# BGU-CS-VIL/DPMMSubClusters.jl

Hardware: AMD Instinct MI355X
Metric: Gibbs iterations/sec, N=10M D=64 NIW (higher is better)
Workload: dtype f32

## Files before the change

### dpmmsubclusters.jl_amd/binding.py

```python
import ctypes
import os
import subprocess

import numpy as np

_HERE = os.path.dirname(os.path.abspath(__file__))
PRIOR_NIW, PRIOR_MULT = 0, 1
MAX_CLUSTERS = 1024

_c_i64p = ctypes.POINTER(ctypes.c_int64)
_c_f32p = ctypes.POINTER(ctypes.c_float)
_c_f64p = ctypes.POINTER(ctypes.c_double)

ABI = [
    ("dpmm_abi_version", ctypes.c_int, []),
    ("dpmm_create", ctypes.c_int, [ctypes.POINTER(ctypes.c_void_p), ctypes.c_int, ctypes.c_int, ctypes.c_int64, ctypes.c_int64, ctypes.c_int, ctypes.c_uint64]),
    ("dpmm_destroy", ctypes.c_int, [ctypes.c_void_p]),
    ("dpmm_last_error", ctypes.c_char_p, [ctypes.c_void_p]),
    ("dpmm_upload_points", ctypes.c_int, [ctypes.c_void_p, _c_f32p, ctypes.c_int64]),
    ("dpmm_upload_points_device", ctypes.c_int, [ctypes.c_void_p, ctypes.c_void_p, ctypes.c_int64]),
    ("dpmm_upload_points_npy", ctypes.c_int, [ctypes.c_void_p, ctypes.c_void_p, ctypes.c_int, ctypes.c_int64, ctypes.c_int]),
    ("dpmm_upload_points_csc", ctypes.c_int, [ctypes.c_void_p, _c_i64p, _c_i64p, _c_f32p, ctypes.c_int]),
    ("dpmm_init_labels", ctypes.c_int, [ctypes.c_void_p, ctypes.c_int, ctypes.c_uint32]),
    ("dpmm_set_labels", ctypes.c_int, [ctypes.c_void_p, _c_i64p, _c_i64p]),
# ... 20 lines not shown
    ("dpmm_mult_master_draw", ctypes.c_int, [ctypes.c_void_p, ctypes.c_uint32, ctypes.c_int, ctypes.c_int, ctypes.c_void_p, ctypes.c_void_p]),
    ("dpmm_mult_master_draws", ctypes.c_int, [ctypes.c_void_p, ctypes.c_int, ctypes.c_void_p]),
    ("dpmm_mult_master_put_rows", ctypes.c_int, [ctypes.c_void_p, ctypes.c_void_p, ctypes.c_int]),
    ("dpmm_mult_master_pairs_ahead", ctypes.c_int, [ctypes.c_void_p, ctypes.c_int, ctypes.c_void_p, ctypes.c_void_p, ctypes.c_int]),
    ("dpmm_mult_master_marginals", ctypes.c_int, [ctypes.c_void_p, ctypes.c_int, ctypes.POINTER(ctypes.c_void_p), ctypes.POINTER(ctypes.c_void_p), ctypes.POINTER(ctypes.c_int)]),
    ("dpmm_mult_master_rows_on_demand", ctypes.c_int, [ctypes.c_void_p, ctypes.c_int]),
    ("dpmm_mult_master_rows_wait", ctypes.c_int, [ctypes.c_void_p]),
    ("dpmm_sweep", ctypes.c_int, [ctypes.c_void_p, ctypes.c_uint32, ctypes.c_int]),
    ("dpmm_packed_stride", ctypes.c_int64, [ctypes.c_void_p]),
    ("dpmm_suffstats_packed_device", ctypes.c_int, [ctypes.c_void_p, _c_i64p, ctypes.c_int, ctypes.c_void_p]),
    ("dpmm_suffstats_packed", ctypes.c_int, [ctypes.c_void_p, _c_i64p, ctypes.c_int, _c_f64p]),
    ("dpmm_unpack_suffstats", ctypes.c_int, [ctypes.c_void_p, ctypes.c_int, _c_f64p, _c_f64p, _c_f64p, _c_f64p]),
    ("dpmm_split", ctypes.c_int, [ctypes.c_void_p, _c_i64p, _c_i64p, ctypes.c_int, ctypes.c_uint32]),
    ("dpmm_merge", ctypes.c_int, [ctypes.c_void_p, _c_i64p, _c_i64p, ctypes.c_int]),
    ("dpmm_remove_empty", ctypes.c_int, [ctypes.c_void_p, _c_i64p, ctypes.c_int]),
    ("dpmm_reset_sublabels", ctypes.c_int, [ctypes.c_void_p, _c_i64p, ctypes.c_int, ctypes.c_uint32]),
    ("dpmm_set_predictive_niw", ctypes.c_int, [ctypes.c_void_p, ctypes.c_int, _c_f32p, _c_f32p, _c_f32p, _c_f32p, _c_f32p]),
    ("dpmm_set_predictive_mult", ctypes.c_int, [ctypes.c_void_p, ctypes.c_int, _c_f32p, _c_f32p]),
    ("dpmm_predict", ctypes.c_int, [ctypes.c_void_p, _c_f32p]),
    ("dpmm_predict_points", ctypes.c_int, [ctypes.c_void_p, _c_i64p, _c_f32p]),
    ("dpmm_set_ground_truth", ctypes.c_int, [ctypes.c_void_p, _c_i64p, ctypes.c_int]),
    ("dpmm_contingency", ctypes.c_int, [ctypes.c_void_p, ctypes.c_int, _c_i64p]),
    ("dpmm_bin_counts", ctypes.c_int, [ctypes.c_void_p, _c_i64p]),
    ("dpmm_smart_project", ctypes.c_int, [ctypes.c_void_p, ctypes.c_int64, _c_f64p, _c_f64p, _c_f64p, _c_i64p]),
    ("dpmm_smart_kmeans_iter", ctypes.c_int, [ctypes.c_void_p, ctypes.c_int64, ctypes.c_double, ctypes.c_double, _c_f64p]),
    ("dpmm_smart_assign", ctypes.c_int, [ctypes.c_void_p, ctypes.c_int64, ctypes.c_double, ctypes.c_double]),
    ("dpmm_debug_loglik", ctypes.c_int, [ctypes.c_void_p, _c_f32p]),
    ("dpmm_sync", ctypes.c_int, [ctypes.c_void_p]),
    ("dpmm_stream", ctypes.c_void_p, [ctypes.c_void_p]),
    ("dpmm_last_sweep_parts_ms", ctypes.c_int, [ctypes.c_void_p, _c_f32p]),
    ("dpmm_last_kernel_ms", ctypes.c_int, [ctypes.c_void_p, _c_f32p, _c_f32p]),
    ("dpmm_debug_counters", ctypes.c_int, [ctypes.c_void_p, ctypes.POINTER(ctypes.c_int64), ctypes.c_int]),
    ("dpmm_debug_sort_tables", ctypes.c_int, [ctypes.c_void_p, ctypes.c_void_p, ctypes.c_void_p, ctypes.c_void_p, ctypes.c_void_p]),
    ("dpmm_debug_set_prelaunch_hook", ctypes.c_int, [ctypes.c_void_p, ctypes.c_void_p]),
    ("dpmm_init_labels_from", ctypes.c_int, [ctypes.c_void_p, ctypes.c_int, ctypes.c_int, ctypes.c_uint32]),
    ("dpmm_set_option", ctypes.c_int, [ctypes.c_void_p, ctypes.c_int, ctypes.c_double]),
    ("dpmm_params_staging", ctypes.c_int, [ctypes.c_void_p, ctypes.c_int] + [ctypes.POINTER(ctypes.c_void_p)] * 6),
    ("dpmm_commit_params", ctypes.c_int, [ctypes.c_void_p, ctypes.c_int]),
    ("dpmm_suffstats_host", ctypes.c_int, [ctypes.c_void_p, _c_i64p, ctypes.c_int, ctypes.POINTER(ctypes.c_void_p)]),
    ("dpmm_step_stats", ctypes.c_int, [ctypes.c_void_p, ctypes.c_uint32, ctypes.POINTER(ctypes.c_void_p), ctypes.POINTER(ctypes.c_void_p)]),
    ("dpmm_debug_subloglik", ctypes.c_int, [ctypes.c_void_p, _c_f32p]),
    ("dpmm_debug_ref_bracket", ctypes.c_int, [ctypes.c_void_p, ctypes.c_int64, ctypes.c_float, _c_f32p, _c_f32p]),
    ("dpmm_debug_pair_ball", ctypes.c_int, [ctypes.c_void_p, _c_f32p, _c_f32p]),
    ("dpmm_debug_pair_ball_sn2", ctypes.c_int, [ctypes.c_void_p, _c_f32p]),
    ("dpmm_debug_norm_cert_points", ctypes.c_int, [ctypes.c_void_p, ctypes.c_int, ctypes.POINTER(ctypes.c_uint8)]),
    ("dpmm_debug_bracket_big", ctypes.c_int, [ctypes.c_void_p, _c_f32p, ctypes.POINTER(ctypes.c_uint32)]),
    ("dpmm_debug_mult_draws_ahead", ctypes.c_int, [ctypes.c_void_p, ctypes.POINTER(ctypes.c_longlong)]),
    ("dpmm_last_sweep_work", ctypes.c_int, [ctypes.c_void_p, ctypes.POINTER(ctypes.c_uint64)]),
    ("dpmm_comm_use_library", ctypes.c_int, [ctypes.c_char_p]),
    ("dpmm_comm_unique_id", ctypes.c_int, [ctypes.c_void_p]),
    ("dpmm_comm_init", ctypes.c_int, [ctypes.c_void_p, ctypes.c_void_p, ctypes.c_int, ctypes.c_int]),
    ("dpmm_comm_init_host", ctypes.c_int, [ctypes.c_void_p, ctypes.c_int, ctypes.c_int, ctypes.c_void_p, ctypes.c_void_p]),
    ("dpmm_comm_info", ctypes.c_int, [ctypes.c_void_p, _c_i64p]),
    ("dpmm_last_comm_ms", ctypes.c_int, [ctypes.c_void_p, _c_f32p, _c_f32p]),
    ("dpmm_comm_destroy", ctypes.c_int, [ctypes.c_void_p]),
    ("dpmm_comm_allgather_host", ctypes.c_int, [ctypes.c_void_p, ctypes.c_void_p, ctypes.c_int64, ctypes.c_void_p]),
]

ABI_TENSOR = [
    ("dpmm_upload_points_strided_device", ctypes.c_int, [ctypes.c_void_p, ctypes.c_void_p, ctypes.c_int, ctypes.c_int64, ctypes.c_int64, ctypes.c_int]),
    ("dpmm_get_points_device", ctypes.c_int, [ctypes.c_void_p, ctypes.c_void_p, ctypes.c_int64]),
    ("dpmm_get_labels_device", ctypes.c_int, [ctypes.c_void_p, ctypes.c_void_p, ctypes.c_void_p]),
    ("dpmm_set_labels_device", ctypes.c_int, [ctypes.c_void_p, ctypes.c_void_p, ctypes.c_void_p]),
    ("dpmm_predict_points_device", ctypes.c_int, [ctypes.c_void_p, ctypes.c_void_p, ctypes.c_void_p]),
]
_c_f64p_in = ctypes.POINTER(ctypes.c_double)
# ... 1215 lines not shown
        self._chk(self._lib.dpmm_debug_loglik(self._h, _p(out, _c_f32p)))
        return out

    def sync(self):
        self._chk(self._lib.dpmm_sync(self._h))

    @property
    def stream(self):
        return self._lib.dpmm_stream(self._h)

    def set_timing(self, on):
        mask = 7 if on is True else int(on)
        self.timing = mask != 0
        self.set_option(OPT_KERNEL_TIMING, float(mask))

    def last_sweep_parts_ms(self):
        out = np.zeros(3, np.float32)
        self._chk(self._lib.dpmm_last_sweep_parts_ms(self._h, _p(out, _c_f32p)))
        return [float(v) for v in out]

    def last_kernel_ms(self):
        if not self.timing:
            raise RuntimeError("kernel timing is off for this Worker (timing=False / set_timing(False)): no events were recorded")
        a = ctypes.c_float(); b = ctypes.c_float()
        self._chk(self._lib.dpmm_last_kernel_ms(self._h, ctypes.byref(a), ctypes.byref(b)))
        return a.value, b.value

    def debug_sort_tables(self):
        perm = np.empty(max(self.n, 1), np.int32); tot = np.empty(2 * self.K, np.int32); start = np.empty(2 * self.K + 1, np.int32)
        ptot = np.zeros(1, np.int32)
        self._chk(self._lib.dpmm_debug_sort_tables(self._h, perm.ctypes.data, tot.ctypes.data, start.ctypes.data, ptot.ctypes.data))
        return perm[:int(ptot[0])].copy(), tot, start

    def debug_counters(self):
        out = (ctypes.c_int64 * 4)()
        self._chk(self._lib.dpmm_debug_counters(self._h, out, 4))
        return list(out)
```

### dpmmsubclusters.jl_amd/csrc/dpmm_api.cpp

```cpp
#include "../../include/dpmm_hip.h"
#include "../../include/dpmm_hip_master.h"
#include "../../include/dpmm_hip_debug.h"
#include "../../include/dpmm_hip_tensor.h"
#include "../../include/dpmm_hip_csc.h"
#include "../../include/dpmm_hip_score.h"
#include "../../include/dpmm_hip_rank.h"
#include "../../include/dpmm_hip_overlap.h"
#include "../../include/dpmm_hip_batchstats.h"
#include "../../include/dpmm_hip_countstats.h"
#include "../../include/dpmm_hip_typicality.h"
#include "../../include/dpmm_hip_explain.h"
#include "../../include/dpmm_hip_holdout.h"
#include "../../include/dpmm_hip_countholdout.h"
#include "../../include/dpmm_hip_trace.h"
#include "../../include/dpmm_hip_missing.h"
#include "../../include/dpmm_hip_impute.h"
#include "../../include/dpmm_hip_regress.h"
#include "../../include/dpmm_hip_regress_draw.h"
#include "../../include/dpmm_hip_regress_cdf.h"
#include "../../include/dpmm_hip_recommend.h"
#include "../../include/dpmm_hip_sample.h"
#include "../../include/dpmm_hip_project.h"

#include <hip/hip_runtime.h>
// ... 15 lines not shown
#include <vector>

#include "dpmm_kernels.h"
#include "project_image.h"
#include "typicality_math.h"
#include "dev_mem.h"

namespace dpmm {
void (*g_prelaunch)(void *) = nullptr;
void *g_prelaunch_arg = nullptr;
}
using namespace dpmm;

static_assert(DPMM_MAX_CLUSTERS == DPMM_MAX_CLUSTERS_K, "header / kernel limits out of sync");

#ifdef DPMM_STAMPS
static unsigned long long *g_dbg = nullptr;
#endif
namespace {
thread_local std::string g_create_error;

int nb_for_dim(int D) { return D <= 16 ? 1 : D <= 32 ? 2 : D <= 64 ? 4 : D <= 128 ? 8 : 16; }
}

struct AccSession {
    bool active = false;
    int K = 0, mode = 0, floor = 0;
    float min_logdens = 0.f;
    unsigned long long gen = 0;
    int use2 = 0;
    float min2 = 0.f;
    bool accumulated = false;
};

struct dpmm_ctx {
    int prior = 0, D = 0, device = 0;
    int64_t n = 0, first = 0, ldx = 0;
    uint64_t seed = 0;
    int NB = 0;
    int tile = 0;
    int64_t ntiles = 0;
    int cus = 256;
    int sweep_grid = 0, sweep_grid_max = 0;
    hipStream_t stream = nullptr;
    hipEvent_t ev[4] = {nullptr, nullptr, nullptr, nullptr};
    hipEvent_t ev_part[2] = {nullptr, nullptr};
    int have_parts = 0;
    bool have_sweep_ev = false, have_stats_ev = false;

    DevBuf<float> dX;
    DevBuf<int32_t> dbins;
    bool have_points = false, have_labels = false;
    DevBuf<int32_t> d_gt;
    int n_gt = 0;
    DevBuf<unsigned long long> d_cont;
    bool have_perm = false;

    int K = 0, Kcap = 0;
    DevBuf<float> d_raw;
    DevBuf<float> d_mu;
    DevBuf<float> d_Rp;
    DevBuf<float> d_mup;
    DevBuf<float> d_cst;
    DevBuf<uint32_t> d_Lp16;
    DevBuf<float> d_raw2, d_Rp2;
    DevBuf<uint32_t> d_Lp16_2;
// ... 183 lines not shown
    uint32_t noise_epoch = 0;
    int noise_nmat = 0, noise_buf = 0;
    bool spec_inflight = false, spec_valid = false;
    uint32_t spec_epoch = 0;
    std::vector<int32_t> spec_slots;
    DevBuf<int32_t> d_jobs, d_dslots;
    PinBuf<int32_t> h_list[4];
    int h_list_next = 0;
    std::vector<int32_t> jobs_shadow, dslots_shadow;
    PinBuf<uint8_t> h_master;
    bool draws_on_device = false;
    DevBuf<unsigned long long> d_work;
    int work_waves = 0;
    long long work_launches = 0;
    float opt_margin = 50.f;
    int opt_prio = 1;
    int opt_queue_rounds = -1;
    int opt_ball = 1;
    DevBuf<uint32_t> d_sp_frag;
    DevBuf<uint32_t> d_refb_big;
    bool have_refb_big = false;
    DevBuf<uint32_t> d_brk_flag;
    DevBuf<float> d_brk_aref;
    DevBuf<float> d_sp_cons;
    PinBuf<uint32_t> h_need;
    int opt_direction = -1;
    bool sp_ready = false, sp_regime = false;
    unsigned sp_count = 0;
    bool sp_last = false;
    int sp_K = -1;
    int sp_cooldown = 0;
    int opt_b3 = 1;
    bool have_b3 = false;
    int opt_chain = 0x7fffffff & ~(8 | 32);
    DevBuf<uint8_t> d_cert_rec;
    int opt_lean_norm_cert = 1;
    int opt_pair_ball = 1;
    bool have_pb = false;
    int opt_lean_dir = 1;
    int opt_master_poll = 1;
    int opt_lean = 1;
    DevBuf<uint32_t> d_hard;
    int hard_flip = 0;
    int perm_nbins = 0;
    PinBuf<uint32_t> h_hard;
    bool sn2_tight = false;
    bool cert_fb = false;
    int cert_cool = 0;
    int lean_off = 0;
    bool lean_ran = false;
    int lean_backoff = 15;
    int opt_bf16scr = 1;
    int opt_bracket = 1;
    int opt_timing = 0;
    int opt_tail = 1, opt_prescreen = -1, opt_ordered = 1, opt_force_f32 = 0, opt_trace = 0, opt_ref_const = 0;
    int64_t opt_stats_items = 0;
    int opt_stats_groups = 0;
    void *comm = nullptr;
    int rank = 0, world = 1;
    dpmm_host_allreduce_fn host_fn = nullptr;
    void *host_user = nullptr;
    PinBuf<char> h_red;
    hipEvent_t ev_comm[4] = {nullptr, nullptr, nullptr, nullptr};
    bool have_comm_ev[2] = {false, false};
    int64_t comm_bytes[2] = {0, 0};
    int64_t comm_calls = 0;
    int comm_timeout_ms = 1800000;
// ... 40 lines not shown
}
static inline void wd_arm(dpmm_ctx *c) {
    std::lock_guard<std::mutex> lk(c->wd_mu);
    c->wd_wait_since.store(steady_ms() | 1, std::memory_order_relaxed);
}
static inline bool wd_disarm(dpmm_ctx *c) {
    std::lock_guard<std::mutex> lk(c->wd_mu);
    c->wd_wait_since.store(0, std::memory_order_relaxed);
    if (c->comm_aborted.load() && !c->abort_reported) { c->abort_reported = true; return true; }
    return false;
}
static inline hipError_t sync_stream(dpmm_ctx *c, hipStream_t st) {
    if (st == c->stream) c->sync_gen += 1;
    if (!c->watchdog || !c->coll_pending) return hipStreamSynchronize(st);
    wd_arm(c);
    hipError_t e = hipStreamSynchronize(st);
    if (wd_disarm(c)) e = hipErrorLaunchTimeOut;
    else if (e == hipSuccess && st == c->stream) c->coll_pending = false;
    return e;
}
static inline hipError_t sync_event(dpmm_ctx *c, hipEvent_t ev) {
    if (!c->watchdog || !c->coll_pending) return hipEventSynchronize(ev);
    wd_arm(c);
    hipError_t e = hipEventSynchronize(ev);
    if (wd_disarm(c)) e = hipErrorLaunchTimeOut;
    return e;
}

static int fail(dpmm_ctx *c, int code, const std::string &msg) {
    if (c) c->err = msg; else g_create_error = msg;
    return code;
}

template <class Buf>
static int regrow(dpmm_ctx *c, Buf &buf, size_t need, const char *who, const char *what, size_t floor = 0) {
    const size_t cap = grow_capacity(need, floor);
    if (buf.alloc(cap) != hipSuccess)
        return fail(c, DPMM_EHIP, std::string(who) + ": out of device memory for the " + what + " (" + std::to_string((unsigned long long)cap) + " bytes)");
    return DPMM_OK;
}
template <class Buf>
static inline int grow(dpmm_ctx *c, Buf &buf, size_t need, const char *who, const char *what, size_t floor = 0) {
    if (need <= buf.bytes) return DPMM_OK;
    HIPCHK(c, sync_stream(c, c->stream));
    return regrow(c, buf, need, who, what, floor);
}
template <typename T>
static int sampler_table(dpmm_ctx *c, DevBuf<T> &dst, const T *src, size_t bytes) {
    HIPCHK(c, dst.alloc(bytes));
    HIPCHK(c, hipMemcpy(dst, src, bytes, hipMemcpyHostToDevice));
    return DPMM_OK;
}
static inline int ensure_pinned(dpmm_ctx *c, size_t bytes) { return grow(c, c->h_pin, bytes, "dpmm", "pinned staging block", (size_t)1 << 20); }

struct UidByValue { char internal[128]; };
namespace {
struct Rccl {
    void *handle = nullptr;
    int (*GetUniqueId)(void *) = nullptr;
    int (*CommInitRank)(void **, int,  UidByValue, int) = nullptr;
    int (*CommDestroy)(void *) = nullptr;
    int (*CommAbort)(void *) = nullptr;
    int (*AllReduce)(const void *, void *, size_t, int, int, void *, hipStream_t) = nullptr;
    int (*AllGather)(const void *, void *, size_t, int, void *, hipStream_t) = nullptr;
    const char *(*GetErrorString)(int) = nullptr;
    std::string err;
// ... 183 lines not shown
    if (prior_kind == DPMM_PRIOR_NIW) {
        c->NB = nb_for_dim(D);
        c->tile = niw_tile_points(c->NB);
        c->slab_stride = niw_slab_stride(D);
        c->packed_stride = 1 + (int64_t)D + (int64_t)D * (D + 1) / 2;
        c->sweep_grid = c->cus * niw_occupancy(c->NB);
        CHK_CREATE(c->d_row_off.alloc(sizeof(int32_t) * (size_t)c->packed_stride));
        CHK_CREATE(c->d_inv_off.alloc(sizeof(int32_t) * (size_t)c->slab_stride));
        CHK_CREATE(launch_niw_row_offsets(c->d_row_off, c->d_inv_off, D, c->packed_stride, c->stream));
    } else {
        c->tile = mult_tile_points();
        c->slab_stride = mult_slab_stride(D);
        c->packed_stride = 1 + (int64_t)D;
        c->sweep_grid = c->cus * 2;
    }
    c->ntiles = (n_local + c->tile - 1) / c->tile;
    if (c->ntiles < c->sweep_grid) c->sweep_grid = (int)std::max<int64_t>(1, c->ntiles);
    c->sweep_grid_max = c->sweep_grid;
    const int64_t target_items = (c->prior == DPMM_PRIOR_NIW && c->D <= 64) ? 16384 : 8192;
    const int64_t min_chunk = (c->prior == DPMM_PRIOR_NIW && c->D <= 64) ? 32 : 256;
    const int64_t target_items2 = (c->prior == DPMM_PRIOR_NIW && c->D <= 64) ? 65536 : target_items;
    c->chunk = (int)std::max<int64_t>(min_chunk, ((n_local + target_items2 - 1) / target_items2 + 3) / 4 * 4);
    c->chunk_dense = c->chunk;
    const size_t nalloc = (size_t)std::max<int64_t>(n_local, 1);
    if (prior_kind == DPMM_PRIOR_NIW) CHK_CREATE(c->dX.alloc(sizeof(float) * nalloc * (size_t)c->ldx));
    CHK_CREATE(c->dbins.alloc(sizeof(int32_t) * nalloc));
    c->sb.tile = n_local <= 4000000 ? SORT_TILE_SMALL : SORT_TILE;
    const int alloc_tile = c->sb.tile;
    c->sort_tile_min = alloc_tile;
    c->nt_sort = (int)((n_local + alloc_tile - 1) / alloc_tile);
    const size_t nbmax = 2 * DPMM_MAX_CLUSTERS;
    CHK_CREATE(c->sort_mem.tile_hist.alloc(sizeof(int32_t) * nbmax * (size_t)std::max(1, c->nt_sort)));
    CHK_CREATE(c->sort_mem.tile_cnt.alloc(sizeof(int32_t) * nbmax * (size_t)std::max(1, c->nt_sort)));
    CHK_CREATE(c->sort_mem.tile_spec.alloc(sizeof(int32_t) * (size_t)STEP_SPEC_MAX_BINS * (size_t)std::max(1, c->nt_sort)));
    CHK_CREATE(c->sort_mem.spec_bins.alloc(sizeof(int32_t) * nalloc));
    CHK_CREATE(c->sort_mem.fast_total.alloc(sizeof(int32_t) * nbmax * FAST_TOTAL_STRIDE));
    CHK_CREATE(hipMemsetAsync(c->sort_mem.fast_total, 0, sizeof(int32_t) * nbmax * FAST_TOTAL_STRIDE, c->stream));
    CHK_CREATE(c->sort_mem.ticket.alloc(sizeof(unsigned)));
    CHK_CREATE(hipMemsetAsync(c->sort_mem.ticket, 0, sizeof(unsigned), c->stream));
    CHK_CREATE(c->sort_mem.prev_lab.alloc(sizeof(uint16_t) * (((size_t)nalloc + SORT_TILE - 1) / SORT_TILE * SORT_TILE)));
    CHK_CREATE(hipMemsetAsync(c->sort_mem.prev_lab, 0xFF, sizeof(uint16_t) * (((size_t)nalloc + SORT_TILE - 1) / SORT_TILE * SORT_TILE), c->stream));
    CHK_CREATE(c->sort_mem.cdirty.alloc(DPMM_MAX_CLUSTERS + 8));
    CHK_CREATE(hipMemsetAsync(c->sort_mem.cdirty, 1, DPMM_MAX_CLUSTERS + 8, c->stream));
    CHK_CREATE(c->sort_mem.cmode.alloc(DPMM_MAX_CLUSTERS));
    CHK_CREATE(hipMemsetAsync(c->sort_mem.cmode, 0, DPMM_MAX_CLUSTERS, c->stream));
    CHK_CREATE(c->sort_mem.bin_total.alloc(sizeof(int32_t) * nbmax));
    CHK_CREATE(c->sort_mem.bin_start.alloc(sizeof(int32_t) * (nbmax + 1)));
    CHK_CREATE(c->sort_mem.item_start.alloc(sizeof(int32_t) * (nbmax + 1)));
    CHK_CREATE(c->sort_mem.perm.alloc(sizeof(int32_t) * nalloc));
    CHK_CREATE(c->sort_mem.bin_sel.alloc(nbmax));
    c->sel_capacity = (int)nbmax;
    CHK_CREATE(c->sort_mem.perm_total.alloc(sizeof(int32_t)));
    sort_view(c);
    CHK_CREATE(c->d_small.alloc(sizeof(int32_t) * 4 * DPMM_MAX_CLUSTERS));
    CHK_CREATE(c->d_counts64.alloc(sizeof(long long) * 2 * DPMM_MAX_CLUSTERS));
    CHK_CREATE(c->d_cside.alloc(DPMM_MAX_CLUSTERS));
    CHK_CREATE(hipMemsetAsync(c->d_cside, 0, DPMM_MAX_CLUSTERS, c->stream));
    if (c->prior == DPMM_PRIOR_NIW && c->NB == 4) {
        CHK_CREATE(c->d_sp_frag.alloc(sizeof(uint32_t) * (size_t)SP_MAXK * SP_FRAG_WORDS));
        CHK_CREATE(c->d_sp_cons.alloc(sizeof(float) * (size_t)SP_MAXK * SP_CONS_FLOATS));
        CHK_CREATE(c->h_need.alloc(sizeof(uint32_t) * 20 * (size_t)std::max(1, c->sweep_grid_max)));
        memset(c->h_need, 0, sizeof(uint32_t) * 20 * (size_t)std::max(1, c->sweep_grid_max));
        if (c->NB == 4) {
            const size_t hw = hard_list_words(n_local);
            CHK_CREATE(c->d_hard.alloc(sizeof(uint32_t) * 2 * hw));
            CHK_CREATE(hipMemsetAsync(c->d_hard, 0, sizeof(uint32_t) * 2 * hw, c->stream));
// ... 201 lines not shown
            if (e == hipSuccess) e = hipMemcpyAsync(n_cp, ncp.data(), sizeof(int64_t) * ((size_t)n + 1), hipMemcpyHostToDevice, c->stream);
            if (e == hipSuccess) e = launch_csc_compact(t_cp, t_rv, t_nz, n, index_base, n_cp, n_ri, n_val, c->stream);
            if (e == hipSuccess) e = sync_stream(c, c->stream);
        }
    } else if (e == hipSuccess) {
        e = hipMemsetAsync(n_cp, 0, sizeof(int64_t), c->stream);
        if (e == hipSuccess) e = sync_stream(c, c->stream);
    }
    if (e != hipSuccess || rc != DPMM_OK) {
        if (e != hipSuccess) return fail(c, DPMM_EHIP, std::string("dpmm_upload_points_csc: ") + hipGetErrorString(e));
        return fail(c, rc, msg);
    }
    t_cp.reset(); t_rv.reset(); t_nz.reset(); t_cnt.reset(); t_bad.reset();
    c->dX.reset(); c->dX8.reset();
    c->d_cp = std::move(n_cp); c->d_ri = std::move(n_ri); c->d_val = std::move(n_val); c->nnz = ncp[n];
    c->x_sparse = 1; c->x_u8 = 0; c->x_bf16_exact = 0; c->repack_pending = false;
    if (int rc2 = set_points_chunk(c, true)) return rc2;
    if (c->have_params && c->d_raw) {
        if (int rc2 = pack_sparse_image(c, c->d_raw, c->d_Rp, c->K)) return rc2;
        c->rp_current = false;
        c->mspec_valid = false;
        HIPCHK(c, sync_stream(c, c->stream));
    }
    c->have_points = true;
    c->cache_force = true;
    c->rows_full_K = -1;
    return DPMM_OK;
}

int dpmm_init_labels(dpmm_ctx *c, int init_clusters, uint32_t epoch) {
    if (!c) return DPMM_EINVAL;
    if (init_clusters < 1 || init_clusters > DPMM_MAX_CLUSTERS) return fail(c, DPMM_ELIMIT, "init_clusters out of range");
    HIPCHK(c, hipSetDevice(c->device));
    if (c->n > 0) HIPCHK(c, launch_init_labels(c->dbins, c->n, c->first, init_clusters, 0, c->seed, epoch, c->stream));
    c->have_labels = true;
    c->rows_full_K = -1;
    return DPMM_OK;
}

int dpmm_init_labels_from(dpmm_ctx *c, int init_clusters, int first_label, uint32_t epoch) {
    if (!c) return DPMM_EINVAL;
    if (first_label < 1 || init_clusters < 1 || first_label - 1 + init_clusters > DPMM_MAX_CLUSTERS) return fail(c, DPMM_ELIMIT, "init_clusters / first_label out of range");
    HIPCHK(c, hipSetDevice(c->device));
    if (c->n > 0) HIPCHK(c, launch_init_labels(c->dbins, c->n, c->first, init_clusters, first_label - 1, c->seed, epoch, c->stream));
    c->have_labels = true;
    c->rows_full_K = -1;
    return DPMM_OK;
}

int dpmm_set_labels(dpmm_ctx *c, const int64_t *labels, const int64_t *sub) {
    if (!c) return DPMM_EINVAL;
    if (!c->have_labels && (!labels || !sub)) return fail(c, DPMM_ESTATE, "first dpmm_set_labels must provide both vectors");
    HIPCHK(c, hipSetDevice(c->device));
    if (c->n == 0) { c->have_labels = true; return DPMM_OK; }
    DevBuf<int64_t> tmp;
    HIPCHK(c, tmp.alloc(sizeof(int64_t) * 2 * (size_t)c->n));
    int rc = DPMM_OK;
    hipError_t e = hipSuccess;
    if (labels) e = hipMemcpyAsync(tmp, labels, sizeof(int64_t) * c->n, hipMemcpyHostToDevice, c->stream);
    if (e == hipSuccess && sub) e = hipMemcpyAsync(tmp + c->n, sub, sizeof(int64_t) * c->n, hipMemcpyHostToDevice, c->stream);
    if (e == hipSuccess) e = launch_bins_from_i64(c->dbins, labels ? tmp.get() : nullptr, sub ? tmp + c->n : nullptr, c->n, c->stream);
    if (e == hipSuccess) e = sync_stream(c, c->stream);
    if (e != hipSuccess) { c->err = std::string("dpmm_set_labels: ") + hipGetErrorString(e); rc = DPMM_EHIP; }
    else c->have_labels = true;
    c->rows_full_K = -1;
    return rc;
}

int dpmm_get_labels(dpmm_ctx *c, int64_t *labels, int64_t *sub) {
    if (!c) return DPMM_EINVAL;
    if (!c->have_labels) return fail(c, DPMM_ESTATE, "labels not initialised");
    HIPCHK(c, hipSetDevice(c->device));
    if (c->n == 0) return DPMM_OK;
    DevBuf<int64_t> tmp;
    HIPCHK(c, tmp.alloc(sizeof(int64_t) * 2 * (size_t)c->n));
    hipError_t e = launch_bins_to_i64(c->dbins, tmp, tmp + c->n, c->n, c->stream);
    if (e == hipSuccess && labels) e = hipMemcpyAsync(labels, tmp, sizeof(int64_t) * c->n, hipMemcpyDeviceToHost, c->stream);
    if (e == hipSuccess && sub) e = hipMemcpyAsync(sub, tmp + c->n, sizeof(int64_t) * c->n, hipMemcpyDeviceToHost, c->stream);
    if (e == hipSuccess) e = sync_stream(c, c->stream);
    if (e != hipSuccess) { c->err = std::string("dpmm_get_labels: ") + hipGetErrorString(e); return DPMM_EHIP; }
    return DPMM_OK;
}

static int check_K(dpmm_ctx *c, int K) {
    if (K < 1) return fail(c, DPMM_EINVAL, "K < 1");
    if (K > DPMM_MAX_CLUSTERS) return fail(c, DPMM_ELIMIT, "K > DPMM_MAX_CLUSTERS");
    return DPMM_OK;
}

struct ParLayout {
    size_t mu = 0, mat = 0, logdet = 0, lr = 0, w = 0, cst = 0, slot = 0, bytes = 0;
};
static ParLayout par_layout(const dpmm_ctx *c, int slots) {
// ... 306 lines not shown
        }
        HIPCHK(c, launch_niw_bracket_big(c->NB, a, c->d_refb_big, c->d_brk_flag, c->d_brk_aref, c->stream));
        a.brk_flag = c->d_brk_flag; a.brk_aref = c->d_brk_aref;
    }
    a.work = table ? nullptr : c->d_work;
    if (!table) { c->work_waves = std::max(c->work_waves, 4 * c->sweep_grid); c->work_launches += 1; }
    a.prio = c->opt_prio; a.queue_rounds = c->opt_queue_rounds;
#ifdef DPMM_STAMPS
    if (!g_dbg) { hipMalloc(&g_dbg, sizeof(unsigned long long) * 16 * 4 * 4096); hipMemset(g_dbg, 0, sizeof(unsigned long long) * 16 * 4 * 4096); }
    a.dbg = g_dbg;
#endif
    return DPMM_OK;
}

static bool lean_this_sweep(dpmm_ctx *c, const NiwSweepArgs &a) {
    const bool lean_ok = c->opt_lean != 0 && c->opt_bracket && a.use_prev && a.screen_margin > 0.f && !a.final_argmax && a.lam == nullptr && c->K > 1 && c->d_hard &&
                         !(c->opt_lean_dir == 0 && c->sp_regime && c->opt_direction != 0 && c->sp_ready);
    if (!lean_ok) return false;
    if (c->lean_off == 0 && c->lean_ran) {
        const int64_t nwt = (c->n + 63) / 64;
        if ((int64_t)c->h_hard[0] * 10 > nwt * 3) { c->lean_off = c->lean_backoff; c->lean_backoff = std::min(2 * c->lean_backoff + 1, 1023); }
        else c->lean_backoff = 15;
        c->lean_ran = false;
    }
    if (c->lean_off > 0) { c->lean_off -= 1; c->h_hard[0] = 0; return false; }
    c->lean_ran = true;
    return true;
}

static int niw_label_store_chain(dpmm_ctx *c, const NiwSweepArgs &a, bool use_lean) {
    const bool parts = (c->opt_timing & 8) != 0 && (c->opt_timing & 1) != 0;
    if (parts && !c->ev_part[0]) for (auto &e : c->ev_part) HIPCHK(c, hipEventCreate(&e));
    NiwLabelStore ls{true};
    if (use_lean) {
        const size_t hw = hard_list_words(c->n);
        uint32_t *mine = c->d_hard + (size_t)c->hard_flip * hw, *other = c->d_hard + (size_t)(c->hard_flip ^ 1) * hw;
        c->hard_flip ^= 1;
        uint32_t *need2 = a.need ? need_lean_settled(c) : nullptr, *need3 = a.need ? need_lean_dir(c) : nullptr;
        const bool al = a.order != nullptr && c->perm_nbins > 0 && c->perm_nbins <= NIW_LEAN_MAX_BINS;
        NiwSweepArgs al_args = a;
        if (!c->opt_lean_dir) { al_args.sp_frag = nullptr; al_args.sp_cons = nullptr; }
        if (c->have_pb && c->opt_pair_ball && al_args.ball) {
            al_args.ball |= NIW_BALL_PAIR_TABLE;
            if (c->opt_lean_norm_cert) al_args.ball |= NIW_BALL_NORM_CERT;
            if (c->opt_lean_norm_cert == 3) al_args.ball |= NIW_BALL_NB_LOOSE;
        }
        c->cert_fb = need2 != nullptr && (al_args.ball & NIW_BALL_NORM_CERT) != 0 && !(al_args.sp_frag && al_args.sp_cons);
#ifndef DPMM_STAMPS
        al_args.cert_points = c->d_cert_rec;
#endif
        HIPCHK(c, launch_niw_lean(al_args, mine, need2, other, al ? c->sb.bin_start : nullptr, al ? c->perm_nbins : 0, need3, c->sweep_grid, c->stream));
        if (parts) HIPCHK(c, hipEventRecord(c->ev_part[0], c->stream));
        ls.tile_list = mine;
        ls.list_len = c->h_hard;
    }
    HIPCHK(c, launch_niw_sweep(c->NB, a, c->sweep_grid, c->stream, ls));
    if (parts) HIPCHK(c, hipEventRecord(c->ev_part[1], c->stream));
    c->have_parts = parts ? (use_lean ? 2 : 1) : 0;
    if (!ls.tile_list) HIPCHK(c, launch_niw_sub(a, nullptr, nullptr, c->sweep_grid, c->stream));
    return DPMM_OK;
}

static int run_sweep(dpmm_ctx *c, uint32_t epoch, int final_argmax, float *table, int64_t table_stride, int64_t p0 = 0, int64_t np = -1) {
    if (!c->have_points || !c->have_params) return fail(c, DPMM_ESTATE, "sweep needs points and parameters");
    HIPCHK(c, hipSetDevice(c->device));
    if (c->n == 0) return DPMM_OK;
    const bool ranged = np >= 0;
    if (ranged && (!table || p0 < 0 || p0 % c->tile != 0 || np == 0 || p0 + np > c->n)) return fail(c, DPMM_EINVAL, "run_sweep: bad point range");
    const int64_t rn = ranged ? np : c->n;
    const int64_t rtiles = ranged ? (np + c->tile - 1) / c->tile : c->ntiles;
    const int rgrid = ranged ? (int)std::min<int64_t>(c->sweep_grid, rtiles) : c->sweep_grid;
    if (c->prior == DPMM_PRIOR_NIW && !table) {
        if (!c->work_zeroed) HIPCHK(c, hipMemsetAsync(c->d_work, 0, sizeof(unsigned long long) * DPMM_WORK_SLOTS, c->stream));
        c->work_zeroed = false;
    }
    if (!table && (c->opt_timing & 1)) HIPCHK(c, hipEventRecord(c->ev[0], c->stream));
    if (c->prior == DPMM_PRIOR_NIW) {
        NiwSweepArgs a{};
        if (int rc = niw_sweep_args(c, a, epoch, final_argmax, table, table_stride, ranged, p0, rn, rtiles)) return rc;
        const bool b3 = c->NB == 4 && c->have_b3 && c->opt_b3 && !table && !c->predictive && a.tail != nullptr;
        if (b3) {
            if (int rc = niw_label_store_chain(c, a, lean_this_sweep(c, a))) return rc;
        } else {
            HIPCHK(c, launch_niw_sweep(c->NB, a, rgrid, c->stream));
            if (!table) c->have_parts = 0;
        }
    } else {
        MultSweepArgs a{};
        a.X = (ranged && c->dX) ? c->dX + p0 * c->ldx : c->dX; a.ldx = c->ldx; a.n = rn; a.first_index = c->first + p0; a.D = c->D; a.K = c->K;
        a.logp = c->d_Rp; a.cst = c->d_cst;
        a.scratch = table ? table : c->d_scratch;
        a.scratch_stride = table ? table_stride : c->scratch_stride;
// ... 120 lines not shown
    if (c->n == 0) return DPMM_OK;
    const int64_t stride = c->ntiles * c->tile;
    const int rows = (c->prior == DPMM_PRIOR_NIW) ? c->K : 3 * c->K;
    DevBuf<float> table;
    HIPCHK(c, table.alloc(sizeof(float) * (size_t)rows * (size_t)stride));
    int rc = run_sweep(c, 0, 0, table, stride);
    if (rc == DPMM_OK) {
        const size_t src_pitch = sizeof(float) * stride * (c->prior == DPMM_PRIOR_MULT ? 3 : 1);
        hipError_t e = hipMemcpy2DAsync(out, sizeof(float) * c->n, table, src_pitch, sizeof(float) * c->n,
                                        (size_t)c->K, hipMemcpyDeviceToHost, c->stream);
        if (e == hipSuccess) e = sync_stream(c, c->stream);
        if (e != hipSuccess) { c->err = std::string("dpmm_debug_loglik: ") + hipGetErrorString(e); rc = DPMM_EHIP; }
        else if (c->opt_ref_const && c->prior == DPMM_PRIOR_NIW && !c->predictive) {
            const float k2pi = (float)(-0.5 * (double)c->D * (double)c->D * log(2.0 * M_PI));
            for (size_t i = 0; i < (size_t)c->K * (size_t)c->n; ++i) out[i] += k2pi;
        }
    }
    return rc;
}

int64_t dpmm_packed_stride(const dpmm_ctx *c) { return c ? c->packed_stride : 0; }

static inline int ensure_out(dpmm_ctx *c, size_t bytes) {
    if (bytes <= c->h_out.bytes) return DPMM_OK;
    HIPCHK(c, sync_stream(c, c->stream));
    c->rows_late = false;
    return regrow(c, c->h_out, bytes, "dpmm", "pinned statistics rows", (size_t)1 << 20);
}

static int flush_undo(dpmm_ctx *c) {
    if (!c->undo_pending) return DPMM_OK;
    c->undo_pending = false;
    const uint8_t *flags = reinterpret_cast<const uint8_t *>(c->d_out.get()) + sizeof(double) * 2 * (size_t)c->K * (size_t)c->packed_stride;
    HIPCHK(c, launch_niw_undo_reset(c->dbins, c->n, c->K, flags, c->d_cside, c->stream));
    return DPMM_OK;
}
static int run_stats(dpmm_ctx *c, const int64_t *idx, int n_idx, bool with_reset = false, uint32_t reset_epoch = 0, uint8_t *flags_to = nullptr,
                     bool *flags_sent = nullptr) {
    if (!c->have_points || !c->have_labels || c->K < 1) return fail(c, DPMM_ESTATE, "suffstats need points, labels and parameters (K)");
    HIPCHK(c, hipSetDevice(c->device));
    const int nbins = 2 * c->K;
    c->marg_valid = false;
    c->mspec_valid = false;
    const bool one_auto = c->packed_stride <= 4096;
    const bool one_coll = with_reset && comm_attached(c) && (c->opt_one_collective < 0 ? one_auto : c->opt_one_collective != 0);
    c->last_pass_one_collective = one_coll;
    if (c->opt_timing & 2) HIPCHK(c, hipEventRecord(c->ev[2], c->stream));
    if (idx) {
        c->h_sel.assign(nbins, 0);
        for (int j = 0; j < n_idx; ++j) {
            if (idx[j] < 1 || idx[j] > c->K) return fail(c, DPMM_EINVAL, "cluster index out of range");
            c->h_sel[2 * (idx[j] - 1)] = 1;
            c->h_sel[2 * (idx[j] - 1) + 1] = 1;
        }
        if (int rc = ensure_pinned(c, nbins + 8)) return rc;
        HIPCHK(c, sync_stream(c, c->stream));
        memcpy(c->h_pin, c->h_sel.data(), nbins);
        HIPCHK(c, launch_copy_bytes(c->sb.bin_sel, c->h_pin, nbins, c->stream));
        c->sel_all_ones = 0;
    } else if (with_reset && c->n > 0 && c->opt_derive) {
    } else if (c->sel_all_ones < nbins) {
        HIPCHK(c, hipMemsetAsync(c->sb.bin_sel, 1, c->sel_capacity, c->stream));
        c->sel_all_ones = c->sel_capacity;
    }
    bool derive = false;
    StatsArgs a{};
    a.X = c->dX; a.ldx = c->ldx; a.n = c->n; a.D = c->D; a.nbins = nbins; a.chunk = c->chunk;
    a.max_items = (int)((c->n + c->chunk - 1) / c->chunk) + nbins;
    a.range_groups = c->opt_stats_groups;
    a.sb = c->sb; a.slabs = c->d_slabs; a.slab_stride = c->slab_stride; a.out = (one_coll && c->prior == DPMM_PRIOR_NIW) ? c->d_red : c->d_out; a.packed_stride = c->packed_stride; a.row_off = c->d_row_off; a.inv_off = c->d_inv_off;
    if (with_reset && c->n > 0) {
        const bool fold_reset = (c->opt_chain & 8) != 0 && (c->n >= 4000000 || (c->opt_chain & 32) != 0) && nbins <= STEP_SPEC_MAX_BINS &&
                                c->sb.tile_spec != nullptr && c->sb.spec_bins != nullptr;
        HIPCHK(c, launch_step_hist(c->dbins, c->n, nbins, c->sb, c->stream, fold_reset ? 1 : 0, c->first, c->seed, reset_epoch));
        const long long *gc = nullptr;
        if (comm_attached(c) && !one_coll) {
            HIPCHK(c, launch_widen_counts(c->sb.fast_total, FAST_TOTAL_STRIDE, c->d_counts64, nbins, c->stream));
            if (int rc = comm_allreduce(c, c->d_counts64, nbins, 0)) return rc;
            gc = c->d_counts64;
        }
        uint8_t *flags = reinterpret_cast<uint8_t *>(c->d_out.get()) + sizeof(double) * (size_t)nbins * (size_t)c->packed_stride;
        if (!fold_reset) HIPCHK(c, launch_step_reset(c->dbins, c->n, c->first, nbins, c->sb, gc, flags, c->K, c->seed, reset_epoch, one_coll ? c->d_cside : nullptr, c->stream));
        derive = c->opt_derive != 0;
        const int force_all = (c->cache_force || c->cache_K != c->K) ? 1 : 0;
        const StepReset rs{gc, flags, c->K, one_coll ? c->d_cside : nullptr, c->first, c->seed, reset_epoch};
        HIPCHK(c, launch_step_scan_scatter(c->dbins, a, derive ? 1 : 0, force_all, c->opt_chain & 1, fold_reset ? &rs : nullptr, c->stream));
        if (derive) { c->sel_all_ones = 0; c->cache_force = false; c->cache_K = c->K; }
    } else {
        if (c->n > 0) {
            HIPCHK(c, launch_sort_by_bin(c->dbins, c->n, nbins, c->sb, c->stream));
        } else {
            HIPCHK(c, hipMemsetAsync(c->sb.bin_total, 0, sizeof(int32_t) * nbins, c->stream));
        }
        if (with_reset && one_coll) {
            HIPCHK(c, hipMemsetAsync(c->d_cside, 0, (size_t)c->K, c->stream));
        } else if (with_reset) {
            const long long *gc = nullptr;
            if (comm_attached(c)) {
                HIPCHK(c, launch_widen_counts(c->sb.bin_total, 1, c->d_counts64, nbins, c->stream));
                if (int rc = comm_allreduce(c, c->d_counts64, nbins, 0)) return rc;
                gc = c->d_counts64;
            }
            uint8_t *flags = reinterpret_cast<uint8_t *>(c->d_out.get()) + sizeof(double) * (size_t)nbins * (size_t)c->packed_stride;
            HIPCHK(c, launch_bad_flags(c->sb.bin_total, gc, c->K, flags, c->stream));
        }
        HIPCHK(c, launch_sort_finish(c->dbins, a, c->stream));
    }
    c->have_perm = c->n > 0;
    c->perm_nbins = nbins;
    if (flags_sent) *flags_sent = false;
    if (one_coll) {
        uint8_t *flags = reinterpret_cast<uint8_t *>(c->d_out.get()) + sizeof(double) * (size_t)nbins * (size_t)c->packed_stride;
        const size_t nred = 3 * (size_t)c->K * (size_t)c->packed_stride;
        if (c->n > 0 && c->prior == DPMM_PRIOR_NIW) {
            if (derive) { a.mode = c->sb.cmode; a.cache = c->d_ccache; a.dirty = c->sb.cdirty; a.K = c->K; }
            a.cside = c->d_cside; a.zero2 = flags + c->K;
            HIPCHK(c, launch_niw_stats(a, c->stream));
        } else if (c->n > 0) {
            if (c->x_sparse) HIPCHK(c, launch_mult_stats_sparse(a, sparse_args(c), c->stream));
            else if (c->x_u8) HIPCHK(c, launch_mult_stats_u8(a, c->dX8, c->ld8, c->stream));
            else HIPCHK(c, launch_mult_stats(a, c->stream));
            if (derive) HIPCHK(c, launch_derive_rows(c->d_out, c->d_ccache, c->sb.cmode, c->sb.cdirty, c->packed_stride, c->K, flags, nullptr, c->stream));
// ... 14 lines not shown
        return DPMM_OK;
    }
    const bool ride = derive && flags_to != nullptr && !comm_attached(c);
    const uint8_t *fsrc = reinterpret_cast<const uint8_t *>(c->d_out.get()) + sizeof(double) * (size_t)nbins * (size_t)c->packed_stride;
    if (c->prior == DPMM_PRIOR_NIW) {
        if (derive) {
            a.mode = c->sb.cmode; a.cache = c->d_ccache; a.dirty = c->sb.cdirty; a.K = c->K;
            a.flags_src = ride ? fsrc : nullptr; a.flags_dst = ride ? flags_to : nullptr;
        }
        HIPCHK(c, launch_niw_stats(a, c->stream));
    } else {
        if (c->x_sparse) HIPCHK(c, launch_mult_stats_sparse(a, sparse_args(c), c->stream));
        else if (c->x_u8) HIPCHK(c, launch_mult_stats_u8(a, c->dX8, c->ld8, c->stream));
        else HIPCHK(c, launch_mult_stats(a, c->stream));
        if (derive) HIPCHK(c, launch_derive_rows(c->d_out, c->d_ccache, c->sb.cmode, c->sb.cdirty, c->packed_stride, c->K, fsrc, ride ? flags_to : nullptr, c->stream));
    }
    if (ride && flags_sent) *flags_sent = true;
    if (comm_attached(c)) {
        if (int rc = comm_allreduce(c, c->d_out, (size_t)nbins * (size_t)c->packed_stride, 1)) return rc;
    }
    if (c->opt_timing & 2) HIPCHK(c, hipEventRecord(c->ev[3], c->stream));
    c->have_stats_ev = (c->opt_timing & 2) != 0;
    c->rows_full_K = idx ? -1 : c->K;
    return DPMM_OK;
}

int dpmm_bin_counts(dpmm_ctx *c, int64_t *counts) {
    if (!c || !counts) return DPMM_EINVAL;
    if (!c->have_points || !c->have_labels || c->K < 1) return fail(c, DPMM_ESTATE, "bin counts need points, labels and parameters (K)");
    HIPCHK(c, hipSetDevice(c->device));
    const int nbins = 2 * c->K;
    if (c->n == 0) { for (int b = 0; b < nbins; ++b) counts[b] = 0; return DPMM_OK; }
    if (int rc = ensure_pinned(c, sizeof(int32_t) * nbins)) return rc;
    HIPCHK(c, launch_sort_by_bin(c->dbins, c->n, nbins, c->sb, c->stream));
    HIPCHK(c, launch_copy_bytes(c->h_pin, c->sb.bin_total, sizeof(int32_t) * nbins, c->stream));
    HIPCHK(c, sync_stream(c, c->stream));
    const int32_t *h = reinterpret_cast<const int32_t *>(c->h_pin.get());
    for (int b = 0; b < nbins; ++b) counts[b] = h[b];
    return DPMM_OK;
}

int dpmm_suffstats_packed_device(dpmm_ctx *c, const int64_t *idx, int n_idx, double *d_out) {
    if (!c || !d_out) return DPMM_EINVAL;
    if (int rc = run_stats(c, idx, n_idx)) return rc;
    HIPCHK(c, hipMemcpyAsync(d_out, c->d_out, sizeof(double) * 2 * c->K * (size_t)c->packed_stride, hipMemcpyDeviceToDevice, c->stream));
    HIPCHK(c, sync_stream(c, c->stream));
    return DPMM_OK;
}

int dpmm_suffstats_host(dpmm_ctx *c, const int64_t *idx, int n_idx, const double **packed) {
    if (!c || !packed) return DPMM_EINVAL;
    const size_t out_bytes = sizeof(double) * 2 * (size_t)std::max(c->K, 1) * (size_t)c->packed_stride;
    if (int rc = ensure_out(c, out_bytes + DPMM_MAX_CLUSTERS + 64)) return rc;
    if (int rc = run_stats(c, idx, n_idx)) return rc;
    HIPCHK(c, launch_copy_bytes(c->h_out, c->d_out, out_bytes, c->stream));
    HIPCHK(c, sync_stream(c, c->stream));
    *packed = reinterpret_cast<const double *>(c->h_out.get());
    return DPMM_OK;
}

static int mult_marginals_launch(dpmm_ctx *c);
int dpmm_step_stats(dpmm_ctx *c, uint32_t reset_epoch, const double **packed, const uint8_t **bad) {
    if (!c || !packed || !bad) return DPMM_EINVAL;
    const size_t out_bytes = sizeof(double) * 2 * (size_t)std::max(c->K, 1) * (size_t)c->packed_stride;
    if (int rc = ensure_out(c, out_bytes + DPMM_MAX_CLUSTERS + 64)) return rc;
    const bool maybe_late = c->rows_on_demand && c->marg_req && c->opt_mult_draws_ahead && c->mdraw_seen && c->draws_on_device && c->d_raw2;
// ... 205 lines not shown
            else if (now - drained > std::chrono::seconds(5)) { rc = fail(c, DPMM_EHIP, "posterior records missing 5 s after the stream drained"); break; }
        } else if (q != hipErrorNotReady) { c->err = std::string("hipStreamQuery while waiting for the posteriors: ") + hipGetErrorString(q); rc = DPMM_EHIP; break; }
    }
    if (armed && wd_disarm(c)) {
        c->err = "collective timed out: a peer rank is gone or stuck (communicator aborted after DPMM_OPT_COMM_TIMEOUT_MS)";
        return DPMM_ECOMM;
    }
    if (c->comm_aborted.load(std::memory_order_relaxed) && rc == DPMM_OK && master_records_marked(sm, nrec)) return fail(c, DPMM_ECOMM, "communicator aborted");
    return rc;
}

int dpmm_debug_set_prelaunch_hook(void (*fn)(void *), void *arg) {
    dpmm::g_prelaunch_arg = arg;
    dpmm::g_prelaunch = fn;
    return DPMM_OK;
}

int dpmm_debug_counters(dpmm_ctx *c, int64_t *out, int n) {
    if (!c || !out || n < 1) return DPMM_EINVAL;
    for (int i = 0; i < n; ++i) out[i] = 0;
    out[0] = c->dbg_early_wait;
    return DPMM_OK;
}

int dpmm_debug_sort_tables(dpmm_ctx *c, int32_t *perm, int32_t *bin_total, int32_t *bin_start, int32_t *perm_total) {
    if (!c || !perm || !bin_total || !bin_start || !perm_total) return DPMM_EINVAL;
    if (!c->have_perm || c->K < 1) return fail(c, DPMM_ESTATE, "no statistics pass has sorted the points yet");
    HIPCHK(c, hipSetDevice(c->device));
    HIPCHK(c, hipStreamSynchronize(c->stream));
    HIPCHK(c, hipMemcpy(perm, c->sb.perm, sizeof(int32_t) * (size_t)c->n, hipMemcpyDeviceToHost));
    HIPCHK(c, hipMemcpy(bin_total, c->sb.bin_total, sizeof(int32_t) * 2 * (size_t)c->K, hipMemcpyDeviceToHost));
    HIPCHK(c, hipMemcpy(bin_start, c->sb.bin_start, sizeof(int32_t) * (2 * (size_t)c->K + 1), hipMemcpyDeviceToHost));
    HIPCHK(c, hipMemcpy(perm_total, c->sb.perm_total, sizeof(int32_t), hipMemcpyDeviceToHost));
    return DPMM_OK;
}

int dpmm_step_master_device(dpmm_ctx *c, uint32_t reset_epoch, const int32_t *slots, uint32_t draw_epoch, const uint8_t **bad, const double **small) {
    if (!c || !slots || !bad || !small) return DPMM_EINVAL;
    if (!c->master) return fail(c, DPMM_ESTATE, "dpmm_niw_master_setup first");
    const int K = c->K;
    if (K < 1) return fail(c, DPMM_ESTATE, "no clusters");
    HIPCHK(c, hipSetDevice(c->device));
    int top = 0;
    for (int k = 0; k < K; ++k) {
        if (slots[k] < 0 || slots[k] >= DPMM_MAX_CLUSTERS) return fail(c, DPMM_EINVAL, "slot out of range");
        top = std::max(top, slots[k] + 1);
    }
    if (int rc = noise_flush(c)) return rc;
    if (int rc = master_capacity(c, top, draw_epoch ? K : 0)) return rc;
    if (int rc = spec_join(c)) return rc;
    c->spec_valid = false;
    const size_t out_bytes = sizeof(double) * 2 * (size_t)K * (size_t)c->packed_stride;
    if (int rc = ensure_out(c, DPMM_MAX_CLUSTERS + 64)) return rc;
    const size_t jobs_bytes = (sizeof(int32_t) * 2 * (size_t)K + 63) & ~(size_t)63;
    if (int rc = master_pinned(c, jobs_bytes + sizeof(double) * 3 * DPMM_MASTER_NSCALARS * (size_t)K)) return rc;
    std::vector<int32_t> jobs(2 * (size_t)K);
    for (int k = 0; k < K; ++k) { jobs[2 * k] = k; jobs[2 * k + 1] = slots[k]; }
    if (int rc = device_list(c, c->d_jobs, c->jobs_shadow, jobs.data(), jobs.size())) return rc;
    if (draw_epoch) if (int rc = device_list(c, c->d_dslots, c->dslots_shadow, slots, (size_t)K)) return rc;
    for (int32_t sl : c->apairs_req) if (sl >= top) { c->apairs_req.clear(); break; }
    const int napairs = (int)(c->apairs_req.size() / 2);
    c->apairs_valid = false;
    bool fuse_pairs = true;
    if (napairs > 0) {
        if ((size_t)napairs > c->apairs_cap) {
            HIPCHK(c, sync_stream(c, c->stream));
// ... 501 lines not shown
                    Sr[(size_t)a * D + b] = Sr[(size_t)b * D + a] = vr;
                    Sc[(size_t)a * D + b] = Sc[(size_t)b * D + a] = vl + vr;
                }
        }
    }
    return DPMM_OK;
}

static int upload_idx(dpmm_ctx *c, const int64_t *a, const int64_t *b, int n, int limit) {
    if (n < 0 || n > 2 * DPMM_MAX_CLUSTERS) return fail(c, DPMM_ELIMIT, "index list too long");
    std::vector<int32_t> h((size_t)(b ? 2 : 1) * n);
    for (int j = 0; j < n; ++j) {
        if (a[j] < 1 || a[j] > limit) return fail(c, DPMM_EINVAL, "cluster index out of range");
        h[j] = (int32_t)(a[j] - 1);
        if (b) {
            if (b[j] < 1 || b[j] > limit) return fail(c, DPMM_EINVAL, "cluster index out of range");
            h[n + j] = (int32_t)(b[j] - 1);
        }
    }
    if (int rc = ensure_pinned(c, sizeof(int32_t) * h.size())) return rc;
    HIPCHK(c, sync_stream(c, c->stream));
    memcpy(c->h_pin, h.data(), sizeof(int32_t) * h.size());
    HIPCHK(c, launch_copy_bytes(c->d_small, c->h_pin, sizeof(int32_t) * h.size(), c->stream));
    return DPMM_OK;
}

int dpmm_split(dpmm_ctx *c, const int64_t *idx, const int64_t *new_idx, int n, uint32_t epoch) {
    if (!c) return DPMM_EINVAL;
    if (!c->have_labels) return fail(c, DPMM_ESTATE, "labels not initialised");
    if (n == 0) return DPMM_OK;
    if (!idx || !new_idx) return fail(c, DPMM_EINVAL, "null index list");
    HIPCHK(c, hipSetDevice(c->device));
    if (int rc = upload_idx(c, idx, new_idx, n, DPMM_MAX_CLUSTERS)) return rc;
    if (c->n > 0) HIPCHK(c, launch_split(c->dbins, c->n, c->first, c->d_small, n, c->seed, epoch, c->stream));
    c->rows_full_K = -1;
    return DPMM_OK;
}

int dpmm_merge(dpmm_ctx *c, const int64_t *idx, const int64_t *new_idx, int n) {
    if (!c) return DPMM_EINVAL;
    if (!c->have_labels) return fail(c, DPMM_ESTATE, "labels not initialised");
    if (n == 0) return DPMM_OK;
    if (!idx || !new_idx) return fail(c, DPMM_EINVAL, "null index list");
    HIPCHK(c, hipSetDevice(c->device));
    if (int rc = upload_idx(c, idx, new_idx, n, DPMM_MAX_CLUSTERS)) return rc;
    if (c->n > 0) HIPCHK(c, launch_merge(c->dbins, c->n, c->d_small, n, c->stream));
    c->rows_full_K = -1;
    return DPMM_OK;
}

int dpmm_remove_empty(dpmm_ctx *c, const int64_t *pts_count, int K) {
    if (!c) return DPMM_EINVAL;
    if (!c->have_labels) return fail(c, DPMM_ESTATE, "labels not initialised");
    if (!pts_count || K < 1 || K > DPMM_MAX_CLUSTERS) return fail(c, DPMM_EINVAL, "bad pts_count / K");
    HIPCHK(c, hipSetDevice(c->device));
    std::vector<int32_t> map(DPMM_MAX_CLUSTERS);
    for (int l = 1; l <= DPMM_MAX_CLUSTERS; ++l) {
        int v = l, removed = 0;
        for (int k = 1; k <= K; ++k)
            if (pts_count[k - 1] == 0) {
                if (v > k - removed) v -= 1;
                removed += 1;
            }
        map[l - 1] = v - 1;
    }
    if (int rc = ensure_pinned(c, sizeof(int32_t) * map.size())) return rc;
    HIPCHK(c, sync_stream(c, c->stream));
    memcpy(c->h_pin, map.data(), sizeof(int32_t) * map.size());
    HIPCHK(c, launch_copy_bytes(c->d_small, c->h_pin, sizeof(int32_t) * map.size(), c->stream));
    if (c->n > 0) HIPCHK(c, launch_remap(c->dbins, c->n, c->d_small, c->stream));
    c->rows_full_K = -1;
    return DPMM_OK;
}

int dpmm_reset_sublabels(dpmm_ctx *c, const int64_t *idx, int n, uint32_t epoch) {
    if (!c) return DPMM_EINVAL;
    if (!c->have_labels) return fail(c, DPMM_ESTATE, "labels not initialised");
    HIPCHK(c, hipSetDevice(c->device));
    if (idx) {
        if (n == 0) return DPMM_OK;
        if (int rc = upload_idx(c, idx, nullptr, n, DPMM_MAX_CLUSTERS)) return rc;
    }
    if (c->n > 0) HIPCHK(c, launch_reset_sub(c->dbins, c->n, c->first, idx ? c->d_small : nullptr, idx ? n : 0, c->seed, epoch, c->stream));
    c->rows_full_K = -1;
    return DPMM_OK;
}

static int smart_buffers(dpmm_ctx *c) {
    if (c->d_proj) return DPMM_OK;
    const size_t n = (size_t)std::max<int64_t>(c->n, 1);
    HIPCHK(c, c->d_proj.alloc(sizeof(double) * n));
    HIPCHK(c, c->d_vals.alloc(sizeof(double) * n));
    HIPCHK(c, c->d_smart.alloc(sizeof(double) * (4 * (size_t)smart_groups() + 8 + 2 * (size_t)c->D)));
    return DPMM_OK;
}
static int smart_check(dpmm_ctx *c, int64_t cluster) {
    if (!c->have_points || !c->have_labels) return fail(c, DPMM_ESTATE, "smart split needs points and labels");
    if (cluster < 1 || cluster > DPMM_MAX_CLUSTERS) return fail(c, DPMM_EINVAL, "cluster index out of range");
    return DPMM_OK;
}

int dpmm_smart_project(dpmm_ctx *c, int64_t cluster, const double *v, const double *mu, double *values, int64_t *count) {
    if (!c || !v || !mu || !count) return DPMM_EINVAL;
    if (int rc = smart_check(c, cluster)) return rc;
    HIPCHK(c, hipSetDevice(c->device));
    if (int rc = smart_buffers(c)) return rc;
    *count = 0;
    if (c->n == 0) return DPMM_OK;
    double *d_v = c->d_smart + 4 * (size_t)smart_groups() + 8, *d_mu = d_v + c->D;
    unsigned long long *d_cnt = reinterpret_cast<unsigned long long *>(c->d_smart + 4 * (size_t)smart_groups() + 4);
    HIPCHK(c, hipMemcpyAsync(d_v, v, sizeof(double) * c->D, hipMemcpyHostToDevice, c->stream));
    HIPCHK(c, hipMemcpyAsync(d_mu, mu, sizeof(double) * c->D, hipMemcpyHostToDevice, c->stream));
    HIPCHK(c, hipMemsetAsync(d_cnt, 0, sizeof(unsigned long long), c->stream));
    HIPCHK(c, launch_smart_project(c->dbins, c->dX, c->ldx, c->n, c->D, (int)(cluster - 1), d_v, d_mu, c->d_proj, c->d_vals, d_cnt, c->stream));
    unsigned long long h = 0;
    HIPCHK(c, hipMemcpyAsync(&h, d_cnt, sizeof(h), hipMemcpyDeviceToHost, c->stream));
    HIPCHK(c, sync_stream(c, c->stream));
    *count = (int64_t)h;
    if (values && h > 0) HIPCHK(c, hipMemcpy(values, c->d_vals, sizeof(double) * h, hipMemcpyDeviceToHost));
    return DPMM_OK;
}

int dpmm_smart_kmeans_iter(dpmm_ctx *c, int64_t cluster, double m_lo, double m_hi, double *out4) {
    if (!c || !out4) return DPMM_EINVAL;
    if (int rc = smart_check(c, cluster)) return rc;
    if (!c->d_proj) return fail(c, DPMM_ESTATE, "dpmm_smart_project has not been called");
    HIPCHK(c, hipSetDevice(c->device));
    out4[0] = out4[1] = out4[2] = out4[3] = 0.;
    if (c->n == 0) return DPMM_OK;
    double *d_out = c->d_smart + 4 * (size_t)smart_groups();
    HIPCHK(c, launch_smart_kmeans(c->dbins, c->d_proj, c->n, (int)(cluster - 1), m_lo, m_hi, c->d_smart, d_out, c->stream));
    HIPCHK(c, hipMemcpyAsync(out4, d_out, sizeof(double) * 4, hipMemcpyDeviceToHost, c->stream));
    HIPCHK(c, sync_stream(c, c->stream));
    return DPMM_OK;
}

int dpmm_smart_assign(dpmm_ctx *c, int64_t cluster, double m_lo, double m_hi) {
    if (!c) return DPMM_EINVAL;
    if (int rc = smart_check(c, cluster)) return rc;
    if (!c->d_proj) return fail(c, DPMM_ESTATE, "dpmm_smart_project has not been called");
    HIPCHK(c, hipSetDevice(c->device));
    if (c->n > 0) HIPCHK(c, launch_smart_assign(c->dbins, c->d_proj, c->n, (int)(cluster - 1), m_lo, m_hi, c->stream));
    return DPMM_OK;
}

int dpmm_set_ground_truth(dpmm_ctx *c, const int64_t *gt, int n_gt) {
    if (!c) return DPMM_EINVAL;
    if ((!gt && c->n > 0) || n_gt < 1 || n_gt > 65536) return fail(c, DPMM_EINVAL, "bad ground truth");
    HIPCHK(c, hipSetDevice(c->device));
    if (!c->d_gt) HIPCHK(c, c->d_gt.alloc(sizeof(int32_t) * (size_t)std::max<int64_t>(c->n, 1)));
    HIPCHK(c, c->d_cont.alloc(sizeof(unsigned long long) * (size_t)DPMM_MAX_CLUSTERS * n_gt));
    if (c->n > 0) {
        DevBuf<int64_t> tmp;
        HIPCHK(c, tmp.alloc(sizeof(int64_t) * (size_t)c->n));
        hipError_t e = hipMemcpyAsync(tmp, gt, sizeof(int64_t) * c->n, hipMemcpyHostToDevice, c->stream);
        if (e == hipSuccess) e = launch_i64_to_i32(c->d_gt, tmp, c->n, c->stream);
        if (e == hipSuccess) e = sync_stream(c, c->stream);
        if (e != hipSuccess) { c->err = std::string("dpmm_set_ground_truth: ") + hipGetErrorString(e); return DPMM_EHIP; }
    }
    c->n_gt = n_gt;
    return DPMM_OK;
}

int dpmm_contingency(dpmm_ctx *c, int K, int64_t *counts) {
    if (!c || !counts) return DPMM_EINVAL;
    if (!c->d_gt || !c->have_labels) return fail(c, DPMM_ESTATE, "contingency needs labels and dpmm_set_ground_truth");
    if (int rc = check_K(c, K)) return rc;
    HIPCHK(c, hipSetDevice(c->device));
    const size_t bytes = sizeof(unsigned long long) * (size_t)K * c->n_gt;
    if (int rc = ensure_pinned(c, bytes)) return rc;
    HIPCHK(c, hipMemsetAsync(c->d_cont, 0, bytes, c->stream));
    if (c->n > 0) HIPCHK(c, launch_contingency(c->dbins, c->d_gt, c->n, K, c->n_gt, c->d_cont, c->stream));
    HIPCHK(c, launch_copy_bytes(c->h_pin, c->d_cont, bytes, c->stream));
    HIPCHK(c, sync_stream(c, c->stream));
// ... 19 lines not shown
void *dpmm_stream(dpmm_ctx *c) { return c ? (void *)c->stream : nullptr; }

int dpmm_set_option(dpmm_ctx *c, int option, double value) {
    if (!c) return DPMM_EINVAL;
    switch (option) {
        case DPMM_OPT_SCREEN_MARGIN: if (!(value >= 0)) return fail(c, DPMM_EINVAL, "margin < 0"); c->opt_margin = (float)value; return DPMM_OK;
        case DPMM_OPT_TAIL_SCREEN: c->opt_tail = value != 0; return DPMM_OK;
        case DPMM_OPT_PRESCREEN: c->opt_prescreen = value < 0 ? -1 : (value != 0); return DPMM_OK;
        case DPMM_OPT_ORDERED_SWEEP: c->opt_ordered = value != 0; return DPMM_OK;
        case DPMM_OPT_MULT_FORCE_F32:
            if (c->have_points) return fail(c, DPMM_ESTATE, "DPMM_OPT_MULT_FORCE_F32 must be set before the points are uploaded");
            c->opt_force_f32 = value != 0; return DPMM_OK;
        case DPMM_OPT_STATS_ITEMS:
            if (c->Kcap > 0) return fail(c, DPMM_ESTATE, "DPMM_OPT_STATS_ITEMS must be set before the first parameters / K");
            if (value >= 1) c->chunk_dense = c->chunk = (int)std::max<int64_t>((c->prior == DPMM_PRIOR_NIW && c->D <= 64) ? 32 : 256, ((c->n + (int64_t)value - 1) / (int64_t)value + 3) / 4 * 4);
            if (c->x_sparse) return set_points_chunk(c, true);
            return DPMM_OK;
        case DPMM_OPT_STATS_GROUPS: c->opt_stats_groups = value > 0 ? (int)value : 0; return DPMM_OK;
        case DPMM_OPT_TRACE_SLOW: c->opt_trace = value != 0; return DPMM_OK;
        case DPMM_OPT_LOGLIK_REF_CONST: c->opt_ref_const = value != 0; return DPMM_OK;
        case DPMM_OPT_WAVE_PRIO: c->opt_prio = value != 0; return DPMM_OK;
        case DPMM_OPT_MULT_DRAWS_AHEAD: c->opt_mult_draws_ahead = value != 0; c->mspec_valid = false; return DPMM_OK;
        case DPMM_OPT_SWEEP_QUEUE_ROUNDS: c->opt_queue_rounds = value < 0 ? -1 : (int)value; return DPMM_OK;
        case DPMM_OPT_BALL_SCREEN: c->opt_ball = value != 0; return DPMM_OK;
        case DPMM_OPT_STATS_DERIVE: c->opt_derive = value != 0; c->cache_force = true; return DPMM_OK;
        case DPMM_OPT_NOISE_AHEAD: c->opt_noise_ahead = value < 0 ? -1 : (value != 0); return DPMM_OK;
        case DPMM_OPT_REF_BRACKET: c->opt_bracket = value != 0; return DPMM_OK;
        case DPMM_OPT_COMM_TIMEOUT_MS: c->comm_timeout_ms = value > 0 ? (int)std::min(value, 2.0e9) : 0; return DPMM_OK;
        case DPMM_OPT_BF16_SCREENS: c->opt_bf16scr = value != 0; return DPMM_OK;
        case DPMM_OPT_MASTER_POLL: c->opt_master_poll = value != 0; return DPMM_OK;
        case DPMM_OPT_PAIR_BALL: c->opt_pair_ball = value != 0; if (!c->opt_pair_ball) c->have_pb = false; return DPMM_OK;
        case DPMM_OPT_LEAN_NORM_CERT: c->opt_lean_norm_cert = (value == 2 || value == 3) ? value : (value != 0); c->cert_cool = 0; c->cert_fb = false; return DPMM_OK;
        case DPMM_OPT_LEAN_DIRECTION: c->opt_lean_dir = value != 0; c->lean_off = 0; c->lean_backoff = 15; c->lean_ran = false; return DPMM_OK;
        case DPMM_OPT_CHAIN_FUSION: c->opt_chain = value < 0 ? (0x7fffffff & ~(8 | 32)) : (int)value; return DPMM_OK;
        case DPMM_OPT_LEAN_TILES: c->opt_lean = value != 0; c->lean_off = 0; c->lean_backoff = 15; c->lean_ran = false; return DPMM_OK;
        case DPMM_OPT_B3_SUBLABELS: c->opt_b3 = value != 0; if (!c->opt_b3) c->have_b3 = false; return DPMM_OK;
        case DPMM_OPT_DIRECTION_SCREEN:
            c->opt_direction = value < 0 ? -1 : (value != 0);
            if (c->opt_direction == 0) { c->sp_ready = false; c->sp_regime = false; }
            return DPMM_OK;
        case DPMM_OPT_ONE_COLLECTIVE: c->opt_one_collective = value < 0 ? -1 : (value != 0); return DPMM_OK;
        case DPMM_OPT_SORT_TILE: {
            const int t = (int)value;
            if (t != SORT_TILE && t != SORT_TILE_SMALL) return fail(c, DPMM_EINVAL, "DPMM_OPT_SORT_TILE: 512 or 2048");
            if (t < c->sort_tile_min) {
                if (c->n > 16000000) return fail(c, DPMM_ELIMIT, "DPMM_OPT_SORT_TILE: 512-point tiles are limited to shards of 16e6 points");
                HIPCHK(c, hipSetDevice(c->device));
                HIPCHK(c, sync_stream(c, c->stream));
                const int nt = (int)((c->n + t - 1) / t);
                const size_t nbmax = 2 * DPMM_MAX_CLUSTERS;
                DevBuf<int32_t> th, tc, tsp;
                if (th.alloc(sizeof(int32_t) * nbmax * (size_t)std::max(1, nt)) != hipSuccess || tc.alloc(sizeof(int32_t) * nbmax * (size_t)std::max(1, nt)) != hipSuccess ||
                    tsp.alloc(sizeof(int32_t) * (size_t)STEP_SPEC_MAX_BINS * (size_t)std::max(1, nt)) != hipSuccess)
                    return fail(c, DPMM_EHIP, "DPMM_OPT_SORT_TILE: out of device memory for the 512-point tile tables");
                c->sort_mem.tile_hist = std::move(th); c->sort_mem.tile_cnt = std::move(tc); c->sort_mem.tile_spec = std::move(tsp);
                sort_view(c);
                c->nt_sort = nt; c->sort_tile_min = t;
            }
            c->sb.tile = t; return DPMM_OK;
        }
        case DPMM_OPT_KERNEL_TIMING:
            c->opt_timing = (int)value & 15;
            if (!(c->opt_timing & 1)) c->have_sweep_ev = false;
            if (!(c->opt_timing & 2)) c->have_stats_ev = false;
            if (!(c->opt_timing & 4)) c->have_comm_ev[0] = c->have_comm_ev[1] = false;
            return DPMM_OK;
        case DPMM_OPT_SWEEP_GRID:
            if (value > 0) c->sweep_grid = (int)std::min<double>(std::min<double>(value, (double)c->sweep_grid_max), (double)std::max<int64_t>(1, c->ntiles));
            return DPMM_OK;
        case DPMM_OPT_MULT_NO_U8:
            if (c->have_points) return fail(c, DPMM_ESTATE, "DPMM_OPT_MULT_NO_U8 must be set before the points are uploaded");
            c->opt_no_u8 = value != 0; return DPMM_OK;
        case DPMM_OPT_SCORE_TABLE_MB: c->opt_score_mb = (value < 0 || value != value) ? 128.0 : value; return DPMM_OK;
        case DPMM_OPT_SCORE_MISSING:
            if (value != 0 && c->prior != DPMM_PRIOR_NIW) return fail(c, DPMM_EINVAL, "DPMM_OPT_SCORE_MISSING: the Multinomial prior has no missing features");
            c->opt_score_missing = value != 0; return DPMM_OK;
        case DPMM_OPT_TYPICALITY_GAPS:
            if (value != 0 && c->prior != DPMM_PRIOR_NIW) return fail(c, DPMM_EINVAL, "DPMM_OPT_TYPICALITY_GAPS: the Multinomial prior has no missing features");
            c->opt_typ_gaps = value != 0; return DPMM_OK;
        default: return fail(c, DPMM_EINVAL, "unknown option");
    }
}

int dpmm_last_sweep_work(dpmm_ctx *c, uint64_t *out16) {
    if (!c || !out16) return DPMM_EINVAL;
    HIPCHK(c, hipSetDevice(c->device));
    HIPCHK(c, sync_stream(c, c->stream));
    std::vector<unsigned long long> h((size_t)DPMM_WORK_PER_WAVE * (size_t)c->work_waves);
// ... 573 lines not shown
    } else if (c->dX) {
        HIPCHK(c, launch_points_readback(d_out, ld_out, c->dX, c->ldx, nullptr, 0, c->n, c->D, c->stream));
    } else if (c->x_u8 && c->dX8) {
        HIPCHK(c, launch_points_readback(d_out, ld_out, nullptr, 0, c->dX8, c->ld8, c->n, c->D, c->stream));
    } else return fail(c, DPMM_ESTATE, std::string(fn) + ": the context holds no point storage");
    HIPCHK(c, sync_stream(c, c->stream));
    return DPMM_OK;
}

int dpmm_get_labels_device(dpmm_ctx *c, int64_t *d_labels, int64_t *d_sub) {
    static const char *fn = "dpmm_get_labels_device";
    if (!c) return tensor_no_ctx(fn);
    if (!c->have_labels) return fail(c, DPMM_ESTATE, "labels not initialised");
    HIPCHK(c, hipSetDevice(c->device));
    if (c->n == 0 || (!d_labels && !d_sub)) return DPMM_OK;
    const uint64_t bytes = sizeof(int64_t) * (uint64_t)c->n;
    if (d_labels) if (int rc = check_device_extent(c, fn, "d_labels", d_labels, bytes, sizeof(int64_t))) return rc;
    if (d_sub) if (int rc = check_device_extent(c, fn, "d_sub", d_sub, bytes, sizeof(int64_t))) return rc;
    HIPCHK(c, launch_bins_to_i64(c->dbins, d_labels, d_sub, c->n, c->stream));
    HIPCHK(c, sync_stream(c, c->stream));
    return DPMM_OK;
}

int dpmm_set_labels_device(dpmm_ctx *c, const int64_t *d_labels, const int64_t *d_sub) {
    static const char *fn = "dpmm_set_labels_device";
    if (!c) return tensor_no_ctx(fn);
    if (!c->have_labels && (!d_labels || !d_sub)) return fail(c, DPMM_ESTATE, "first dpmm_set_labels_device must provide both vectors");
    HIPCHK(c, hipSetDevice(c->device));
    if (c->n == 0) { c->have_labels = true; return DPMM_OK; }
    const uint64_t bytes = sizeof(int64_t) * (uint64_t)c->n;
    if (d_labels) if (int rc = check_device_extent(c, fn, "d_labels", d_labels, bytes, sizeof(int64_t))) return rc;
    if (d_sub) if (int rc = check_device_extent(c, fn, "d_sub", d_sub, bytes, sizeof(int64_t))) return rc;
    if (d_labels || d_sub) {
        HIPCHK(c, launch_bins_from_i64(c->dbins, d_labels, d_sub, c->n, c->stream));
        HIPCHK(c, sync_stream(c, c->stream));
    }
    c->have_labels = true;
    c->rows_full_K = -1;
    return DPMM_OK;
}

int dpmm_predict_points_device(dpmm_ctx *c, int64_t *d_labels, float *d_probs) {
    static const char *fn = "dpmm_predict_points_device";
    if (!c) return tensor_no_ctx(fn);
    if (!c->predictive) return fail(c, DPMM_ESTATE, "dpmm_predict_points_device needs dpmm_set_predictive_* first");
    if (!c->have_points || !c->have_params) return fail(c, DPMM_ESTATE, "predict needs points and parameters");
    HIPCHK(c, hipSetDevice(c->device));
    if (c->n == 0) return DPMM_OK;
    if (!d_labels) return fail(c, DPMM_EINVAL, std::string(fn) + ": d_labels is null");
    if (int rc = check_device_extent(c, fn, "d_labels", d_labels, sizeof(int64_t) * (uint64_t)c->n, sizeof(int64_t))) return rc;
    if (d_probs) if (int rc = check_device_extent(c, fn, "d_probs", d_probs, sizeof(float) * (uint64_t)c->n * (uint64_t)c->K, sizeof(float))) return rc;
    const int64_t stride = c->ntiles * c->tile;
    const int rstep = (c->prior == DPMM_PRIOR_NIW) ? 1 : 3;
    DevBuf<float> table;
    HIPCHK(c, table.alloc(sizeof(float) * (size_t)(rstep * c->K) * (size_t)stride));
    int rc = run_sweep(c, 0, 0, table, stride);
    if (rc == DPMM_OK) {
        hipError_t e = launch_predict_finish(table, stride, rstep, c->n, c->K, d_labels, d_probs, c->stream);
        if (e == hipSuccess) e = sync_stream(c, c->stream);
        if (e != hipSuccess) { c->err = std::string(fn) + ": " + hipGetErrorString(e); rc = DPMM_EHIP; }
    }
    return rc;
}

static int score_table_slab(dpmm_ctx *c, int *rstep_out, int64_t *P_out) {
    const int rstep = (c->prior == DPMM_PRIOR_NIW) ? 1 : 3;
// ... 1774 lines not shown
```

### dpmmsubclusters.jl_amd/csrc/dpmm_kernels.h

```cpp
#pragma once
#include <hip/hip_runtime.h>
#include <stddef.h>
#include <stdint.h>
#include "stats_ranges.h"

#define DPMM_MAX_CLUSTERS_K 1024

namespace dpmm {


constexpr int DPMM_WORK_QUEUES = 8;
constexpr int DPMM_WORK_SLOTS = 8 + 16 * DPMM_WORK_QUEUES;
constexpr int DPMM_WORK_PER_WAVE = 8;
constexpr int REFB_FRAGS = 6, REFB_WORDS = REFB_FRAGS * 256;
constexpr int B3_WORDS = 3 * REFB_WORDS;
constexpr int B3_DVEC = 64;

enum NiwBall : int {
    NIW_BALL_ON = 1,
    NIW_BALL_PAIR_TABLE = 2,
    NIW_BALL_NORM_CERT = 4,
    NIW_BALL_NB_LOOSE = 8,
};
enum NiwScreens : int {
    NIW_SCR_ON = 1,
    NIW_SCR_DIR_FIRST = 2,
};

struct NiwSweepArgs {
    const float *X;
    int64_t ldx;
    int64_t n;
    int64_t first_index;
    int64_t ntiles;
    int K;
    const float *Rp;
    const float *mup;
    const float *cst;
    union {
        const float *tdf;
        const uint32_t *tile_list;
    };
    float *scratch;
    int64_t scratch_stride;
    int scratch_by_tile;
    int labels_only;
    int32_t *bins;
    const int32_t *order_total;
    const int32_t *order;
    uint64_t seed;
    uint32_t epoch;
    int final_argmax;
    float screen_margin;
    const float *tail;
    int tail_g;
    int ball;
    int bf16scr;
    int bracket;
    const float *lam;
    union {
        const float *mdist;
        uint32_t *list_len;
    };
    int screen_lds;
    int use_prev;
    int lds_rows;
    union {
        const uint32_t *sp_frag;
        const uint32_t *brk_flag;
    };
    union {
        const float *sp_cons;
        const float *brk_aref;
    };
    uint32_t *need;
    union {
        unsigned long long *dbg;
        uint8_t *cert_points;
    };
    int queue_rounds;
    int prio;
    unsigned long long *work;
};
static_assert(sizeof(NiwSweepArgs) == 256, "NiwSweepArgs: frozen size");
static_assert(offsetof(NiwSweepArgs, tdf) == 72 && offsetof(NiwSweepArgs, tile_list) == 72, "NiwSweepArgs: frozen layout");
static_assert(offsetof(NiwSweepArgs, ball) == 164 && offsetof(NiwSweepArgs, bf16scr) == 168, "NiwSweepArgs: frozen layout");
static_assert(offsetof(NiwSweepArgs, mdist) == 184 && offsetof(NiwSweepArgs, list_len) == 184, "NiwSweepArgs: frozen layout");
static_assert(offsetof(NiwSweepArgs, sp_frag) == 208 && offsetof(NiwSweepArgs, brk_flag) == 208, "NiwSweepArgs: frozen layout");
static_assert(offsetof(NiwSweepArgs, sp_cons) == 216 && offsetof(NiwSweepArgs, brk_aref) == 216, "NiwSweepArgs: frozen layout");
static_assert(offsetof(NiwSweepArgs, dbg) == 232 && offsetof(NiwSweepArgs, cert_points) == 232, "NiwSweepArgs: frozen layout");
static_assert(offsetof(NiwSweepArgs, work) == 248, "NiwSweepArgs: frozen layout");

struct NiwLabelStore {
    bool store_labels = false;
    const uint32_t *tile_list = nullptr;
    uint32_t *list_len = nullptr;
};

int niw_tile_points(int NB);
int niw_occupancy(int NB);
hipError_t launch_niw_sweep(int NB, const NiwSweepArgs &a, int grid, hipStream_t s, const NiwLabelStore &ls = {});
hipError_t launch_niw_refb_debug(const NiwSweepArgs &a, int k, float c_override, float *qhi_out, float *q_out, hipStream_t s);
hipError_t launch_niw_screen_prep(const float *R, const float *mu, int D, int K, float *lam, float *dist, const int32_t *slot, hipStream_t s);
hipError_t launch_niw_pack(const float *R, const float *mu, float *Rp, float *mup, int D, int NB, int nmat, float *tail, const float *cst,
                           const int32_t *slot, float *cst_out, unsigned long long *work, hipStream_t s);
constexpr int SP_MAXK = 64, SP_FRAG_WORDS = 4 * 2 * 256, SP_CONS_FLOATS = 3 * 64;
inline bool niw_steady_launch(const NiwSweepArgs &a, bool store_labels) {
    return a.screen_margin > 0.f && (store_labels || !a.tdf) && !a.scratch_by_tile && !a.labels_only && a.K > 1 && a.lam == nullptr && a.tail != nullptr && !a.final_argmax;
}
inline bool niw_dir_screen(const NiwSweepArgs &a) { return a.sp_frag && a.sp_cons && a.bf16scr && a.K <= SP_MAXK; }
inline size_t niw_refb_big_words(int NB) { size_t c = 0; for (int bi = 0; bi < NB; ++bi) c += NB / 2 - bi / 2; return c * 256; }
hipError_t launch_niw_refb_big(const float *Rp, int NB, int K, uint32_t *out, hipStream_t s);
hipError_t launch_niw_bracket_big(int NB, const NiwSweepArgs &a, const uint32_t *refb, uint32_t *tile_flag, float *aref, hipStream_t s);
hipError_t launch_niw_b3_pack(const float *Rp, const float *mup, int K, float *tail, int what, hipStream_t s);
constexpr int PB_MAXK = 256;
#ifndef DPMM_PB_NORM_SQUARINGS
#define DPMM_PB_NORM_SQUARINGS 3
#endif
constexpr int PB_NORM_SQUARINGS = DPMM_PB_NORM_SQUARINGS;
inline size_t niw_pair_ball_floats(size_t K) { return K <= (size_t)PB_MAXK ? K * K + 2 * K : 0; }
inline size_t niw_pair_ball_offset(size_t K) { return 32 * ((K + 1) >> 1) + 16 * K + (size_t)REFB_WORDS * K + 3 * K * (size_t)B3_WORDS + 3 * K * (size_t)B3_DVEC; }
inline size_t niw_tail_floats(size_t cap) {
    return 16 * (cap + 2) + 16 * cap + (size_t)REFB_WORDS * cap + 3 * cap * (size_t)B3_WORDS + 3 * cap * (size_t)B3_DVEC + niw_pair_ball_floats(cap < (size_t)PB_MAXK ? cap : (size_t)PB_MAXK);
}
hipError_t launch_niw_b3_debug(const NiwSweepArgs &a, float *out, hipStream_t s);
hipError_t launch_niw_sub(const NiwSweepArgs &a, const uint32_t *list, uint32_t *count_out, int grid, hipStream_t s);
constexpr int NIW_LEAN_MAX_BINS = 256;
hipError_t launch_niw_lean(const NiwSweepArgs &a, uint32_t *list, uint32_t *need2, uint32_t *other_list, const int32_t *bin_start, int nbins, uint32_t *need3, int grid, hipStream_t s);
hipError_t launch_niw_direction(const float *Rp, const float *mup, const float *cst, int D, int K, uint32_t *frag, float *cons, hipStream_t s);

struct MultSweepArgs {
    const float *X;
    int64_t ldx;
    int64_t n;
    int64_t first_index;
    int D;
    int K;
    const float *logp;
    const float *cst;
    float *scratch;
    int64_t scratch_stride;
    int scratch_by_tile;
    int labels_only;
    int32_t *bins;
    uint64_t seed;
    uint32_t epoch;
    int final_argmax;
    int use_prev;
    const int32_t *order;
    const int32_t *order_total;
};
hipError_t launch_mult_sweep(const MultSweepArgs &a, int grid, hipStream_t s);
hipError_t launch_mult_pack(const float *logp, float *Lp, int rows, int64_t ldx, hipStream_t s);
int mult_tile_points();
hipError_t launch_bf16_exact_check(const float *X, int64_t nwords, int *d_flag, hipStream_t s);
size_t mult_pack_bf16_words(int rows, int64_t ldx);
hipError_t launch_mult_pack_bf16(const float *logp, uint32_t *Lp16, int rows, int64_t ldx, hipStream_t s);
hipError_t launch_mult_sweep_bf16(const MultSweepArgs &a, const uint32_t *Lp16, int grid, hipStream_t s);
hipError_t launch_u8_convert(const float *X, int64_t ldx, int D, int64_t n, uint8_t *X8, int64_t ld8, int *d_flag, hipStream_t s);
size_t mult_pack_u8_words(int rows, int64_t ld8);
hipError_t launch_mult_pack_u8(const float *logp, uint32_t *Lp8, int rows, int64_t ldx, int64_t ld8, hipStream_t s);
// ... 491 lines not shown
constexpr int SORT_TILE_SMALL = 512;
constexpr int FAST_TOTAL_STRIDE = 32;

struct SortBufs {
    int tile;
    int32_t *tile_hist;
    int32_t *tile_cnt;
    int32_t *spec_bins;
    int32_t *tile_spec;
    int32_t *fast_total;
    unsigned *ticket;
    uint16_t *prev_lab;
    uint8_t *cdirty;
    uint8_t *cmode;
    int32_t *bin_total;
    int32_t *bin_start;
    int32_t *perm;
    int32_t *item_start;
    uint8_t *bin_sel;
    int32_t *perm_total;
};

hipError_t launch_sort_by_bin(const int32_t *bins, int64_t n, int nbins, const SortBufs &b, hipStream_t s);
constexpr int STEP_SPEC_MAX_BINS = 512;
struct StepReset { const long long *global_counts; uint8_t *flags; int K; uint8_t *cside; int64_t first; uint64_t seed; uint32_t epoch; };
hipError_t launch_step_hist(const int32_t *bins, int64_t n, int nbins, const SortBufs &b, hipStream_t s, int spec = 0, int64_t first = 0, uint64_t seed = 0, uint32_t epoch = 0);
hipError_t launch_step_reset(int32_t *bins, int64_t n, int64_t first, int nbins, const SortBufs &b, const long long *global_counts, uint8_t *flags,
                             int K, uint64_t seed, uint32_t epoch, uint8_t *cside, hipStream_t s);
hipError_t launch_onecoll_rows(const double *rows, double *red, int64_t stride, int K, const uint8_t *cside, uint8_t *flags, hipStream_t s);
hipError_t launch_niw_finalize_rows(const double *red, double *out, int64_t stride, int K, const uint8_t *cside, uint8_t *flags, uint8_t *flags_host, hipStream_t s);
hipError_t launch_niw_undo_reset(int32_t *bins, int64_t n, int K, const uint8_t *flags, const uint8_t *cside, hipStream_t s);
struct StatsArgs;
hipError_t launch_sort_finish(const int32_t *bins, const StatsArgs &a, hipStream_t s);
hipError_t launch_step_scan_scatter(int32_t *bins, const StatsArgs &a, int derive, int force_all, int fused_starts, const StepReset *rs, hipStream_t s);
hipError_t launch_derive_rows(double *out, double *cache, const uint8_t *mode, uint8_t *dirty, int64_t stride, int K, const uint8_t *flags_src,
                              uint8_t *flags_dst, hipStream_t s);

struct StatsArgs {
    const float *X;
    int64_t ldx;
    int64_t n;
    int D;
    int nbins;
    int chunk;
    int max_items;
    int range_groups;
    SortBufs sb;
    double *slabs;
    int64_t slab_stride;
    double *out;
    int64_t packed_stride;
    const int32_t *row_off;
    const int32_t *inv_off;
    const uint8_t *mode;
    double *cache;
    uint8_t *dirty;
    const uint8_t *flags_src; uint8_t *flags_dst; int K;
    const uint8_t *cside; uint8_t *zero2;
};
int64_t niw_slab_stride(int D);
hipError_t launch_niw_row_offsets(int32_t *row_off, int32_t *inv_off, int D, int64_t packed_stride, hipStream_t s);
int64_t mult_slab_stride(int D);
hipError_t launch_niw_stats(const StatsArgs &a, hipStream_t s);
hipError_t launch_mult_stats(const StatsArgs &a, hipStream_t s);
hipError_t launch_mult_stats_u8(const StatsArgs &a, const uint8_t *X8, int64_t ld8, hipStream_t s);

#define DPMM_MULT_MASTER_MAXD 16384
// ... 44 lines not shown
```

### dpmmsubclusters.jl_amd/csrc/niw_device.h

```cpp
#pragma once
#include "dpmm_device.h"
#include "dpmm_kernels.h"

namespace dpmm {

typedef float f32x4 __attribute__((ext_vector_type(4)));

template <int NB>
__host__ __device__ constexpr int pair_base(int bi) {
    return bi * NB - (bi * (bi - 1)) / 2;
}

typedef float f32x2 __attribute__((ext_vector_type(2)));
struct TailPair { f32x2 v[16]; };
__device__ __forceinline__ TailPair tail_load_pair(const float *tail, int pair) {
    typedef const float __attribute__((address_space(4))) *cfp4;
    const cfp4 P = (cfp4)(tail + (size_t)pair * 32);
    TailPair T;
#pragma unroll
    for (int q = 0; q < 16; ++q) T.v[q] = (f32x2){P[2 * q], P[2 * q + 1]};
    return T;
}
__device__ __forceinline__ unsigned tail_pair_far(const TailPair &T, const f32x4 &xt, float thr) {
    const f32x2 x0 = (f32x2){xt.x, xt.x}, x1 = (f32x2){xt.y, xt.y}, x2 = (f32x2){xt.z, xt.z}, x3 = (f32x2){xt.w, xt.w};
// ... 124 lines not shown
__device__ __forceinline__ unsigned long long direction_far_core(const uint32_t *__restrict__ frag, const float *__restrict__ cons, const u32x4_t (&zb)[NG][2],
                                                                 const float (&nz)[NG], const float (&thr)[NG], int lane, int g, int K) {
    unsigned long long far = 0ull;
    const int nblk = (K + 15) >> 4;
    for (int blk = 0; blk < nblk; ++blk) {
        const u32x4_t a0 = reinterpret_cast<const u32x4_t *>(frag)[(2 * blk) * 64 + lane], a1 = reinterpret_cast<const u32x4_t *>(frag)[(2 * blk + 1) * 64 + lane];
        const f32x4 cB = *reinterpret_cast<const f32x4 *>(cons + 16 * blk + 4 * g), cE = *reinterpret_cast<const f32x4 *>(cons + 64 + 16 * blk + 4 * g),
                    cK = *reinterpret_cast<const f32x4 *>(cons + 128 + 16 * blk + 4 * g);
        bool ok[4] = {true, true, true, true};
        const f32x4 tau = cB * 0.02f;
#pragma unroll
        for (int n = 0; n < NG; ++n) {
            f32x4 sv = __builtin_amdgcn_mfma_f32_16x16x32_bf16(__builtin_bit_cast(bf16x8_t, a0), __builtin_bit_cast(bf16x8_t, zb[n][0]), (f32x4){0.f, 0.f, 0.f, 0.f}, 0, 0, 0);
            sv = __builtin_amdgcn_mfma_f32_16x16x32_bf16(__builtin_bit_cast(bf16x8_t, a1), __builtin_bit_cast(bf16x8_t, zb[n][1]), sv, 0, 0, 0);
#pragma unroll
            for (int r = 0; r < 4; ++r) {
                float t = __builtin_fmaf(-cE[r], nz[n], fabsf(sv[r] + cB[r]));
                t = t >= tau[r] ? t : 0.f;
                const float ub = __builtin_fmaf(-0.4995f * t, t, cK[r]);
                ok[r] = ok[r] && (ub < thr[n]);
            }
        }
#pragma unroll
        for (int r = 0; r < 4; ++r) {
            const unsigned long long m = __ballot(ok[r]);
#pragma unroll
            for (int gg = 0; gg < 4; ++gg)
                if (((m >> (16 * gg)) & 0xFFFFull) == 0xFFFFull) far |= 1ull << (16 * blk + 4 * gg + r);
        }
    }
    return K >= 64 ? far : far & ((1ull << K) - 1ull);
}

}
```

### dpmmsubclusters.jl_amd/csrc/niw_lean.hip

```cpp
#include "dpmm_device.h"
#include "dpmm_kernels.h"
#include "niw_device.h"
#include "niw_b3.h"

namespace dpmm {

__global__ __launch_bounds__(256) void niw_b3_pack_kernel(const float *__restrict__ Rp, const float *__restrict__ mup, float *__restrict__ tail, int K, int y0, int tight) {
    constexpr int NP = 10;
    uint32_t *img = const_cast<uint32_t *>(b3_images(tail, K));
    float *dvec = const_cast<float *>(b3_offsets(tail, K));
    const int k = blockIdx.x >> 1, j = 3 * k + 1 + (blockIdx.x & 1);
    const float *Rj = Rp + (size_t)j * NP * 256;
    auto elem = [&](int row, int col) -> float {
        const int bi = row >> 4, t = col >> 4;
        if (t < bi) return 0.f;
        const int pair = pair_base<4>(bi) + (t - bi);
        const int ln = (row & 15) + 16 * ((col & 15) >> 2);
        return Rj[(size_t)pair * 256 + ln * 4 + (col & 3)];
    };
    const int yy = (int)blockIdx.y + y0;
    if (yy == 4) {
        if (blockIdx.x & 1) return;
        const float *Rk = Rp + (size_t)(3 * k) * NP * 256;
        auto elemR = [&](int row, int col) -> float {
// ... 24 lines not shown
}
hipError_t launch_niw_b3_pack(const float *Rp, const float *mup, int K, float *tail, int what, hipStream_t s) {
    const bool pb = (what & 2) && K >= 2 && K <= PB_MAXK;
    if (K < 1 || !((what & 1) || pb)) return hipSuccess;
    const int y0 = (what & 1) ? 0 : 4, ny = (pb ? 5 : 4) - y0;
    DPMM_LAUNCH(niw_b3_pack_kernel, dim3(2 * K, ny), dim3(256), 0, s, Rp, mup, tail, K, y0, (what & 4) ? 1 : 0);
    return hipGetLastError();
}

__global__ __launch_bounds__(256) void niw_b3_debug_kernel(NiwSweepArgs A, float *__restrict__ out) {
    const int lane = threadIdx.x & 63, ci = lane & 15, g = lane >> 4;
    const int64_t wbase = ((int64_t)blockIdx.x * 4 + (threadIdx.x >> 6)) * 64;
    if (wbase >= A.n) return;
    const int myp32 = wbase + lane < A.n ? (int)(wbase + lane) : -1;
    for (int k = 0; k < A.K; ++k) {
        f32x4 x[4][4], mk[4];
        gather_x64(A.X, A.ldx, myp32, ci, g, x);
        b3_mean(A.mup, k, g, mk);
        B3Z Z;
        b3_convert(x, mk, Z);
        float bl, br;
        const B3Head H = b3_head(A.tail, A.cst, A.K, k, lane, g);
        b3_eval(A.tail, A.K, k, Z, H, lane, g, bl, br);
        if (myp32 >= 0) { out[(int64_t)(2 * k) * A.n + myp32] = bl; out[(int64_t)(2 * k + 1) * A.n + myp32] = br; }
    }
}
hipError_t launch_niw_b3_debug(const NiwSweepArgs &a, float *out, hipStream_t s) {
    if (!a.tail || a.n <= 0) return hipErrorInvalidValue;
    DPMM_LAUNCH(niw_b3_debug_kernel, dim3((unsigned)((a.n + 255) / 256)), dim3(256), 0, s, a, out);
    return hipGetLastError();
}


template <bool LISTED>
__global__ __launch_bounds__(256, 2) void niw_sub_kernel(NiwSweepArgs A, const uint32_t *__restrict__ list, uint32_t *__restrict__ count_out) {
    if (LISTED && count_out && blockIdx.x == 0 && threadIdx.x == 0) *count_out = list[0];
    const int lane = threadIdx.x & 63, ci = lane & 15, g = lane >> 4;
    const bool use_order = A.order != nullptr && *A.order_total == (int32_t)A.n;
    const int64_t nwtiles = (A.n + 63) / 64;
    const int64_t count = LISTED ? (int64_t)list[0] : nwtiles;
    const int wave_id = (int)blockIdx.x * 4 + (threadIdx.x >> 6), nwaves = (int)gridDim.x * 4;
    unsigned nw_b3 = 0;
    auto span_words = [&](int64_t i, uint32_t &w0, uint32_t &w1) {
        w0 = 0u; w1 = 0xffffffffu;
        if (i >= count) return;
        if constexpr (LISTED) { w0 = list[1 + 2 * i]; w1 = list[2 + 2 * i]; }
        else { const int64_t e = A.n - 64 * i; w0 = (uint32_t)(64 * i); w1 = (uint32_t)(e < 64 ? e : 64); }
    };
    auto pack_span = [](uint32_t w0, uint32_t w1) -> int64_t { return w1 == 0xffffffffu ? (int64_t)-1 : (((int64_t)w0 << 7) | (int64_t)w1); };
    auto label_of = [&](int bin) -> int { const int zz = bin >> 1; return (unsigned)zz < (unsigned)A.K ? zz : -1; };
    uint32_t sa, sb, sa2, sb2;
    span_words(wave_id, sa, sb);
    span_words((int64_t)wave_id + nwaves, sa2, sb2);
    int64_t t_next = pack_span(sa, sb);
    int nx_p = -1, nx_z = -1;
    if (t_next >= 0) {
        const int64_t pos = (t_next >> 7) + lane;
        if (lane < (int)(t_next & 127)) { nx_p = use_order ? A.order[pos] : (int)pos; nx_z = label_of(A.bins[nx_p]); }
    }
    for (int64_t idx = wave_id; idx < count; idx += nwaves) {
        t_next = pack_span(sa2, sb2);
        const int myp32 = nx_p;
        const int z = nx_z;
        int pf_p = -1, pf_bin = -1;
        const bool has_next = t_next >= 0 && lane < (int)(t_next & 127);
        bool bin_asked = false;
        if (has_next) {
            const int64_t posn = (t_next >> 7) + lane;
            pf_p = use_order ? A.order[posn] : (int)posn;
        }
        span_words(idx + 2 * (int64_t)nwaves, sa2, sb2);
        float u_sub = 0.f;
        if (z >= 0) u_sub = u01(philox4x32_10(A.seed, (uint64_t)(A.first_index + myp32), A.epoch, STREAM_SWEEP).v[1]);
        float b0 = -INFINITY, b1 = -INFINITY;
        unsigned long long todo = __ballot(z >= 0);
        while (todo) {
            const int leader = __ffsll((long long)todo) - 1;
            const int k = __builtin_amdgcn_readfirstlane(__shfl(z, leader));
            todo &= ~__ballot(z == k);
            f32x4 x[4][4], mk[4];
            gather_x64(A.X, A.ldx, myp32, ci, g, x);
            b3_mean(A.mup, k, g, mk);
            const B3Head H = b3_head(A.tail, A.cst, A.K, k, lane, g);
            __builtin_amdgcn_sched_barrier(0);
            B3Z Z;
            b3_convert(x, mk, Z);
            if (!bin_asked) {
                int q = pf_p;
                asm volatile("" : "+v"(q));
                if (has_next) pf_bin = A.bins[q];
                bin_asked = true;
            }
            float bl, br;
            b3_eval(A.tail, A.K, k, Z, H, lane, g, bl, br);
            if (z == k) { b0 = bl; b1 = br; }
            nw_b3 += 2;
        }
        if (z >= 0) A.bins[myp32] = 2 * z + draw2(b0, b1, u_sub);
        if (!bin_asked && has_next) pf_bin = A.bins[pf_p];
        nx_p = pf_p; nx_z = has_next ? label_of(pf_bin) : -1;
        asm volatile("" : "+v"(nx_z));
    }
    if (A.work && lane == 0) A.work[DPMM_WORK_SLOTS + (size_t)wave_id * DPMM_WORK_PER_WAVE + 7] += (unsigned long long)nw_b3 << 32;
}
hipError_t launch_niw_sub(const NiwSweepArgs &a, const uint32_t *list, uint32_t *count_out, int grid, hipStream_t s) {
    if (!a.tail || a.n <= 0) return hipErrorInvalidValue;
    if (list) DPMM_LAUNCH(niw_sub_kernel<true>, dim3(grid), dim3(256), 0, s, a, list, count_out);
    else DPMM_LAUNCH(niw_sub_kernel<false>, dim3(grid), dim3(256), 0, s, a, list, count_out);
    return hipGetLastError();
}

__device__ __forceinline__ void ref_bracket_planes(const u32x4_t (&a)[6], const B3Z &Z, float (&qhi)[4]) {
    const u32x4_t absm = (u32x4_t){0x7fff7fffu, 0x7fff7fffu, 0x7fff7fffu, 0x7fff7fffu};
#pragma unroll
    for (int n0 = 0; n0 < 4; n0 += 2) {
        float part[2] = {0.f, 0.f};
#pragma unroll
        for (int bi = 0; bi < 4; ++bi) {
            f32x4 y[2], e[2];
#pragma unroll
            for (int h = 0; h < 2; ++h) { y[h] = (f32x4){0.f, 0.f, 0.f, 0.f}; e[h] = (f32x4){0.f, 0.f, 0.f, 0.f}; }
#pragma unroll
            for (int sl = 0; sl < 2; ++sl) {
                const int f = bi == 0 ? sl : (bi == 1 ? 2 + sl : (sl == 1 ? bi + 2 : -1));
                if (f < 0) continue;
                const u32x4_t aa = a[f] & absm;
#pragma unroll
                for (int h = 0; h < 2; ++h) {
                    const u32x4_t zb = Z.p[n0 + h][sl][0];
                    y[h] = __builtin_amdgcn_mfma_f32_16x16x32_bf16(__builtin_bit_cast(bf16x8_t, a[f]), __builtin_bit_cast(bf16x8_t, zb), y[h], 0, 0, 0);
                    e[h] = __builtin_amdgcn_mfma_f32_16x16x32_bf16(__builtin_bit_cast(bf16x8_t, aa), __builtin_bit_cast(bf16x8_t, zb & absm), e[h], 0, 0, 0);
                }
            }
#pragma unroll
            for (int h = 0; h < 2; ++h)
#pragma unroll
                for (int r = 0; r < 4; ++r) {
                    const float t = __builtin_fmaf(REFB_C, e[h][r], fabsf(y[h][r]));
                    part[h] = __builtin_fmaf(t, t, part[h]);
                }
        }
#pragma unroll
        for (int h = 0; h < 2; ++h) {
            const f32x4 tot = __builtin_amdgcn_mfma_f32_16x16x4f32(1.0f, part[h], (f32x4){0.f, 0.f, 0.f, 0.f}, 0, 0, 0);
            qhi[n0 + h] = __builtin_fmaf(tot[0], 1.0001f, 1e-20f);
        }
    }
}

#ifdef DPMM_STAMPS
#define LSTAMP(var) unsigned long long var; do { __builtin_amdgcn_sched_barrier(0); asm volatile("s_memtime %0\n\ts_waitcnt lgkmcnt(0)" : "=s"(var) :: "memory"); __builtin_amdgcn_sched_barrier(0); } while (0)
#else
#define LSTAMP(var)
#endif
template <bool DIR>
__device__ __forceinline__ void niw_lean_body(NiwSweepArgs A, uint32_t *__restrict__ list, uint32_t *__restrict__ need2, uint32_t *__restrict__ other_list,
                                              const int32_t *__restrict__ bin_start, int nbins, uint32_t *__restrict__ need3) {
    if (other_list && blockIdx.x == 0 && threadIdx.x == 0) other_list[0] = 0u;
#ifdef DPMM_STAMPS
    unsigned long long T_x = 0, T_conv = 0, T_br = 0, T_scr = 0, T_u = 0, T_p2 = 0, T_tot = 0; int ntl = 0;
#endif
    const int lane = threadIdx.x & 63, ci = lane & 15, g = lane >> 4;
    const bool use_order = A.order != nullptr && *A.order_total == (int32_t)A.n;
    const int K = A.K;
    const int wave_id = (int)blockIdx.x * 4 + (threadIdx.x >> 6), nwaves = (int)gridDim.x * 4;
    unsigned nw_easy = 0, nw_br = 0, nw_tail = 0, nw_bb = 0, nw_cheap = 0;
    const bool use_dir = DIR && A.sp_frag != nullptr && A.sp_cons != nullptr && A.bf16scr && K >= 3 && K <= SP_MAXK;
    const bool dir_first = use_dir && (A.bf16scr & NIW_SCR_DIR_FIRST) != 0;
    unsigned nw_sp = 0, nw_cand = 0, nw_dcand = 0, nw_dexcl = 0, nw_ctiles = 0;
    constexpr int BALL_LDS_K = 256;
    __shared__ __attribute__((aligned(16))) float ball_lds[BALL_LDS_K * 16];
    const bool ball_in_lds = A.ball && K <= BALL_LDS_K;
    __shared__ float pb_s[PB_MAXK];
    const bool use_pb = !DIR && (A.ball & NIW_BALL_PAIR_TABLE) != 0 && ball_in_lds && K <= PB_MAXK;
    const float *pb_d = pair_ball_table(A.tail, K);
    __shared__ float pb_s0[PB_MAXK], pb_sc[PB_MAXK];
    const bool use_cert = !DIR && use_pb && (A.ball & NIW_BALL_NORM_CERT) != 0;
    if (use_pb) {
        const float *s_own = pb_d + (size_t)K * K + K, *s_nb = (A.ball & (NIW_BALL_NORM_CERT | NIW_BALL_NB_LOOSE)) == NIW_BALL_NORM_CERT ? s_own : s_own - K;
        for (int e = threadIdx.x; e < K; e += 256) { pb_s[e] = s_own[e - K]; pb_sc[e] = s_nb[e]; pb_s0[e] = s_own[e]; }
    }
    if (ball_in_lds) {
        const float *src = ball_records(A.tail, K);
        for (int e = threadIdx.x; e < 16 * K; e += 256) ball_lds[e] = src[e];
    }
    constexpr int MAXB = NIW_LEAN_MAX_BINS;
    __shared__ int tstart_s[MAXB + 2], bstart_s[MAXB + 2], wsum_s[4];
    const bool aligned = bin_start != nullptr && use_order && nbins >= 1 && nbins <= MAXB && bin_start[nbins] == (int32_t)A.n;
    const int nb = aligned ? nbins : 1;
    {
        const int tid = threadIdx.x;
        int c = 0;
        if (tid < nb) {
            const int s0 = aligned ? bin_start[tid] : 0, s1 = aligned ? bin_start[tid + 1] : (int)A.n;
            c = (s1 - s0 + 63) >> 6; bstart_s[tid] = s0;
        }
        if (tid == 0) bstart_s[nb] = (int)A.n;
        int inc = c;
#pragma unroll
        for (int off = 1; off < 64; off <<= 1) { const int v = __shfl_up(inc, off); if (lane >= off) inc += v; }
        if (lane == 63) wsum_s[tid >> 6] = inc;
        __syncthreads();
        const int w = tid >> 6;
        inc += (w > 0 ? wsum_s[0] : 0) + (w > 1 ? wsum_s[1] : 0) + (w > 2 ? wsum_s[2] : 0);
        tstart_s[tid + 1] = inc;
        if (tid == 0) tstart_s[0] = 0;
    }
    __syncthreads();
    const int ntiles_all = __builtin_amdgcn_readfirstlane(tstart_s[nb]);
    int bptr = 0;
    auto span_of = [&](int t, int &p0, int &cn) {
        p0 = 0; cn = 0;
        if (t >= ntiles_all) return;
        while (t >= __builtin_amdgcn_readfirstlane(tstart_s[bptr + 1])) ++bptr;
        p0 = __builtin_amdgcn_readfirstlane(bstart_s[bptr]) + 64 * (t - __builtin_amdgcn_readfirstlane(tstart_s[bptr]));
        const int e = __builtin_amdgcn_readfirstlane(bstart_s[bptr + 1]) - p0;
        cn = e < 64 ? e : 64;
    };
    auto index_at = [&](int p0, int cn) -> int { return lane < cn ? (use_order ? A.order[p0 + lane] : p0 + lane) : -1; };
    int c_p0, c_cn, n_p0, n_cn;
// ... 171 lines not shown
                    ++nw_tail;
                    cand &= ~((unsigned long long)tail_pair_far(tail_load_pair(A.tail, pr), xt, my_thr) << sh);
                }
                if constexpr (DIR) { if (use_dir && !dir_first) { tile_cand = (unsigned)__builtin_popcountll(cand); direction(); } }
                if (A.bf16scr) {
                    const u32x4_t *Rb0 = reinterpret_cast<const u32x4_t *>(refb_records(A.tail, K));
                    while (cand) {
                        const int k = base + __builtin_ctzll(cand);
                        const u32x4_t a5 = Rb0[(size_t)k * (REFB_WORDS / 4) + 64 * 5 + lane];
                        const f32x4 m4 = *reinterpret_cast<const f32x4 *>(A.mup + (size_t)(3 * k) * 64 + 48 + 4 * g);
                        ++nw_bb;
                        if (!bf16_bottom_excludes<4>(a5, x3, m4, A.cst[3 * k], thrb)) break;
                        cand &= cand - 1ull;
                    }
                }
                hard = cand != 0ull;
                if constexpr (DIR) { if (use_dir && !hard) { nw_cand += tile_cand; nw_sp += tile_sp; nw_dcand += tile_dc; nw_dexcl += tile_dx; ++nw_ctiles; } }
            }
            }
        }
#ifdef DPMM_STAMPS
        { LSTAMP(t4); s4 = t4; }
#endif
        if (!hard) {
            H = b3_head(A.tail, A.cst, K, k0, lane, g);
        }
#ifdef DPMM_STAMPS
        { LSTAMP(t5); s5 = t5; }
#endif
        if (hard) {
            if (lane == 0) { const uint32_t at = atomicAdd(&list[0], 1u); list[1 + 2 * at] = (uint32_t)c_p0; list[2 + 2 * at] = (uint32_t)c_cn; }
            if (!bin_asked && lane < n_cn) pf_bin = A.bins[pf_p];
        } else {
            float bl, br;
            b3_eval(A.tail, K, k0, Z, H, lane, g, bl, br);
            if (valid) A.bins[myp32] = 2 * k0 + draw2(bl, br, u_sub);
#ifndef DPMM_STAMPS
            if (cheap && A.cert_points && valid) A.cert_points[myp32] = 1;
#endif
            ++nw_easy;
        }
        nx_p = pf_p; nx_prev = label_of(pf_bin);
        asm volatile("" : "+v"(nx_prev));
        c_p0 = n_p0; c_cn = n_cn;
        span_of(tile + 2 * nwaves, n_p0, n_cn);
#ifdef DPMM_STAMPS
        { LSTAMP(s6); T_x += s1 - s0; T_conv += s2 - s1; T_br += s3 - s2; T_scr += s4 - s3; T_u += s5 - s4; T_p2 += s6 - s5; T_tot += s6 - s0; ++ntl; }
#endif
    }
#ifdef DPMM_STAMPS
    if (A.dbg && lane == 0) {
        unsigned long long *d = A.dbg + (size_t)(8192 + wave_id) * 16;
        d[0] = T_x; d[1] = T_conv; d[2] = T_br; d[3] = T_scr; d[4] = T_u; d[5] = T_p2; d[6] = 0; d[7] = T_tot; d[8] = ntl;
    }
#endif
    if (A.work && lane == 0) {
        unsigned long long *slot = A.work + DPMM_WORK_SLOTS + (size_t)wave_id * DPMM_WORK_PER_WAVE;
        slot[0] += nw_easy; slot[3] += nw_tail; slot[4] += nw_br; slot[5] += nw_bb; slot[7] += ((unsigned long long)(2 * nw_easy) << 32) + nw_sp;
        slot[6] += (unsigned long long)nw_cheap << 32;
    }
    if (need2 && lane == 0) need2[wave_id] = use_dir ? 0u : ((nw_easy < 65535u ? nw_easy : 65535u) | ((nw_cheap < 65535u ? nw_cheap : 65535u) << 16));
    if (need3 && lane == 0) {
        uint32_t word = 0u, yield = 0u;
        if (use_dir) {
            word = ((nw_cand < 65535u ? nw_cand : 65535u) << 16) | (nw_ctiles < 32767u ? nw_ctiles : 32767u) | (dir_first ? 0x8000u : 0u);
            yield = ((nw_dexcl < 65535u ? nw_dexcl : 65535u) << 16) | (nw_dcand < 65535u ? nw_dcand : 65535u);
        }
        need3[2 * wave_id] = word; need3[2 * wave_id + 1] = yield;
    }
}
__global__ __launch_bounds__(256, 2) void niw_lean_kernel(NiwSweepArgs A, uint32_t *__restrict__ list, uint32_t *__restrict__ need2, uint32_t *__restrict__ other_list,
                                                         const int32_t *__restrict__ bin_start, int nbins, uint32_t *__restrict__ need3) {
    niw_lean_body<false>(A, list, need2, other_list, bin_start, nbins, need3);
}
__global__ __launch_bounds__(256, 2) void niw_lean_kernel_dir(NiwSweepArgs A, uint32_t *__restrict__ list, uint32_t *__restrict__ need2, uint32_t *__restrict__ other_list,
                                                             const int32_t *__restrict__ bin_start, int nbins, uint32_t *__restrict__ need3) {
    niw_lean_body<true>(A, list, need2, other_list, bin_start, nbins, need3);
}
hipError_t launch_niw_lean(const NiwSweepArgs &a, uint32_t *list, uint32_t *need2, uint32_t *other_list, const int32_t *bin_start, int nbins, uint32_t *need3, int grid, hipStream_t s) {
    if (!a.tail || a.n <= 0 || !list) return hipErrorInvalidValue;
    if (nbins > NIW_LEAN_MAX_BINS) { bin_start = nullptr; nbins = 0; }
    if (niw_dir_screen(a) && a.K >= 3) DPMM_LAUNCH(niw_lean_kernel_dir, dim3(grid), dim3(256), 0, s, a, list, need2, other_list, bin_start, nbins, need3);
    else DPMM_LAUNCH(niw_lean_kernel, dim3(grid), dim3(256), 0, s, a, list, need2, other_list, bin_start, nbins, need3);
    return hipGetLastError();
}

}
```

### dpmmsubclusters.jl_amd/csrc/niw_sweep.hip

```cpp
#include "dpmm_device.h"
#include "dpmm_kernels.h"
#include "niw_device.h"
#include "niw_b3.h"
#include <cstdlib>
#include <cstring>

namespace dpmm {

template <int NB, int NG, int CH>
struct NiwCfg {
    static constexpr int DP = 16 * NB;
    static constexpr int NP = NB * (NB + 1) / 2;
    static constexpr int MATSZ = NP * 256;
    static constexpr int CAP = NB >= 16 ? 32 : 16;
    __host__ __device__ static constexpr int chunk_row(int c) {
        int r = 0;
        for (int i = 0; i < c; ++i) {
            int p = 0;
            while (r < NB && p + (NB - r) <= CAP) { p += NB - r; ++r; }
        }
        return r;
    }
    __host__ __device__ static constexpr int count_chunks() {
        int c = 0;
// ... 1476 lines not shown
                }
            } else {
                float s = 0.f;
                for (int k = 0; k < K; ++k) s += exp_det(nan_to_ninf(scr[(int64_t)k * sstride]) - m_run);
                const float t = u01(r.v[0]) * s;
                float cw = 0.f;
                z = K - 1;
                for (int k = 0; k < K; ++k) {
                    cw += exp_det(nan_to_ninf(scr[(int64_t)k * sstride]) - m_run);
                    if (!(cw < t)) { z = k; break; }
                }
            }
        }
        if (!FAST && A.labels_only) continue;
        STAMP(s3);
        if constexpr (LIST) {
            if constexpr (NB == 4 && NG == 4) {
                float b0 = -INFINITY, b1 = -INFINITY;
                unsigned long long todo = __ballot(valid);
                while (todo) {
                    const int leader = __ffsll((long long)todo) - 1;
                    const int kk = __builtin_amdgcn_readfirstlane(__shfl(z, leader));
                    todo &= ~__ballot(valid && z == kk);
                    f32x4 mk[4];
                    b3_mean(A.mup, kk, g, mk);
                    const B3Head H = b3_head(A.tail, A.cst, K, kk, lane, g);
                    B3Z Z;
                    b3_convert(x, mk, Z);
                    float bl, br;
                    b3_eval(A.tail, K, kk, Z, H, lane, g, bl, br);
                    if (z == kk) { b0 = bl; b1 = br; }
                    nw_b3l += 2;
                }
                if (valid) A.bins[myp] = 2 * z + draw2(b0, b1, u_sub);
            }
            nx_p = pf_p; nx_bin = pf_bin; nx_tile = tnext < tile_sent ? tnext : -1;
            l_pos = nl_pos; l_end = nl_end;
            continue;
        }
        if constexpr (LSTORE) {
            if (valid) A.bins[myp] = 2 * z;
            nx_p = pf_p; nx_bin = pf_bin; nx_tile = tnext < tile_sent ? tnext : -1;
            if (LIST) { l_pos = nl_pos; l_end = nl_end; }
            continue;
        }

        float b0 = -INFINITY, b1 = -INFINITY;
        unsigned long long todo = __ballot(valid);
        auto next_label = [&]() -> int {
            if (!todo) return -1;
            const int leader = __ffsll((long long)todo) - 1;
            const int kk = __shfl(z, leader);
            todo &= ~__ballot(valid && z == kk);
            return kk;
        };
        int kcur = next_label();
        if (kcur >= 0 && rb0_mat != 3 * kcur + 1)
            load_rb0<NB>(A.Rp + (size_t)(3 * kcur + 1) * MATSZ, A.mup + (size_t)(3 * kcur + 1) * DP, rb0, mu, lane, g);
        while (kcur >= 0) {
            const int knext = next_label();
            const int jl = 3 * kcur + 1, jr = jl + 1, jn = 3 * (knext >= 0 ? knext : 0) + 1;
            const float cl = A.cst[jl], cr = A.cst[jr];
            const float bl = __builtin_fmaf(-0.5f, quad_stream<NB, NG>(A.Rp + (size_t)jl * MATSZ, A.Rp + (size_t)jr * MATSZ,
                                                                          A.mup + (size_t)jr * DP, rb0, mu, x, lane, g, true, tot_all, A.prio), cl);
            const float br = __builtin_fmaf(-0.5f, quad_stream<NB, NG>(A.Rp + (size_t)jr * MATSZ,
                                                                          knext >= 0 ? A.Rp + (size_t)jn * MATSZ : nullptr,
                                                                          A.mup + (size_t)jn * DP, rb0, mu, x, lane, g, true, tot_all, A.prio), cr);
// ... 403 lines not shown
```

### dpmmsubclusters.jl_amd/csrc/suffstats.hip

```cpp
#include <algorithm>
#include <cstdlib>
#include "dpmm_device.h"
#include "dpmm_kernels.h"
#include "stats_ranges.h"

namespace dpmm {

typedef double f64x4 __attribute__((ext_vector_type(4)));
typedef float f32x4 __attribute__((ext_vector_type(4)));

__device__ __forceinline__ void count_chunk(int x, int y, int z, int w, int *cnt, int nbins, int lane) {
    const int b0 = __builtin_amdgcn_readfirstlane(x);
    const bool ex = x == b0, ey = y == b0, ez = z == b0, ew = w == b0;
    const int c0 = __popcll(__ballot(ex)) + __popcll(__ballot(ey)) + __popcll(__ballot(ez)) + __popcll(__ballot(ew));
    if (c0 == 256) {
        if (lane == 0 && (unsigned)b0 < (unsigned)nbins) atomicAdd(&cnt[b0], 256);
        return;
    }
    const int o = !ex ? x : !ey ? y : !ez ? z : w;
    const unsigned long long has = __ballot(!(ex && ey && ez && ew));
    const int b1 = __builtin_amdgcn_readlane(o, __ffsll((long long)has) - 1);
    const bool fx = x == b1, fy = y == b1, fz = z == b1, fw = w == b1;
    const int c1 = __popcll(__ballot(fx)) + __popcll(__ballot(fy)) + __popcll(__ballot(fz)) + __popcll(__ballot(fw));
    if (lane == 0) {
// ... 326 lines not shown
    }
}
__global__ __launch_bounds__(256) void starts_kernel(const int32_t *__restrict__ bin_total, const uint8_t *__restrict__ bin_sel,
                                                     int nbins, int chunk, int32_t *__restrict__ bin_start,
                                                     int32_t *__restrict__ item_start, int32_t *__restrict__ perm_total) {
    __shared__ int pa[256], pb[256];
    starts_body(bin_total, bin_sel, nbins, chunk, bin_start, item_start, perm_total, pa, pb);
}
__global__ __launch_bounds__(256) void starts_step_kernel(int32_t *bin_total, uint8_t *bin_sel, int nbins, int chunk,
                                                          int32_t *__restrict__ bin_start, int32_t *__restrict__ item_start,
                                                          int32_t *__restrict__ perm_total, int32_t *__restrict__ fast_total,
                                                          uint8_t *__restrict__ mode, const uint8_t *__restrict__ dirty, int force_all) {
    __shared__ int part[256], pb[256];
    if (fast_total) for (int b = threadIdx.x; b < nbins; b += 256) fast_total[b * FAST_TOTAL_STRIDE] = 0;
    if (mode) {
        const bool all = force_all || dirty[DPMM_MAX_CLUSTERS_K];
        for (int k = threadIdx.x; k < nbins / 2; k += 256) {
            const int nl = bin_total[2 * k], nr = bin_total[2 * k + 1];
            const int m = (all || dirty[k] || nl + nr == 0) ? 0 : (nl <= nr ? 2 : 1);
            mode[k] = (uint8_t)m;
            bin_sel[2 * k] = m != 1;
            bin_sel[2 * k + 1] = m != 2;
        }
    }
    __syncthreads();
    starts_body(bin_total, bin_sel, nbins, chunk, bin_start, item_start, perm_total, part, pb);
}

struct StepStarts {
    const int32_t *bin_total; uint8_t *bin_sel; int chunk; int32_t *bin_start_out; int32_t *item_start; int32_t *perm_total; int32_t *fast_total;
    uint8_t *mode; const uint8_t *dirty; int force_all;
    const uint8_t *reset_flags; const int32_t *spec_bins;
    const int32_t *tile_cnt;
};
template <int TILE, bool STEP>
__global__ __launch_bounds__(64) void scatter_kernel(int32_t *bins, int64_t n, int nbins, int nt,
                                                     const int32_t *__restrict__ tile_hist,
                                                     const int32_t *__restrict__ bin_start, int32_t *__restrict__ perm, StepStarts st) {
    extern __shared__ int base[];
    const int lane = threadIdx.x;
    int nbits = 0;
    while ((1 << nbits) < nbins) ++nbits;
    uint8_t *const rflag = reinterpret_cast<uint8_t *>(base + nbins);
    bool do_reset = false;
    if constexpr (STEP) {
        if (st.reset_flags && st.reset_flags[nbins >> 1]) {
            bool need = false;
            for (int b = lane; b < nbins; b += 64) {
                const uint8_t f = st.reset_flags[b >> 1];
                if (!(b & 1)) rflag[b >> 1] = f;
                need = need || (f && st.tile_cnt[(int64_t)b * nt + blockIdx.x] > 0);
            }
            do_reset = __any(need);
        }
    }
    if constexpr (STEP) {
        const bool pub = blockIdx.x == 0;
        const bool all = pub && st.mode && (st.force_all || st.dirty[DPMM_MAX_CLUSTERS_K]);
        int carry = 0, icarry = 0;
        for (int b0 = 0; b0 < nbins; b0 += 64) {
            const int b = b0 + lane;
            const int t = b < nbins ? st.bin_total[b] : 0;
            int inc = t;
#pragma unroll
            for (int off = 1; off < 64; off <<= 1) { const int v = __shfl_up(inc, off); if (lane >= off) inc += v; }
            const int excl = carry + inc - t;
// ... 46 lines not shown
        if ((unsigned)b >= (unsigned)nbins) b = -1;
        if constexpr (STEP) {
            if (do_reset && b >= 0 && rflag[b >> 1]) {
                b = st.spec_bins[i];
                bins[i] = b;
            }
        }
        const bool valid = b >= 0;
        unsigned long long m = __ballot(valid);
        const int bfirst = __builtin_amdgcn_readfirstlane(b);
        if (!__all(b == bfirst)) {
            const unsigned long long m0 = __ballot(b == bfirst), rest = m & ~m0;
            const int bsecond = __shfl(b, rest ? __ffsll((long long)rest) - 1 : 0);
            const unsigned long long m1 = __ballot(valid && b == bsecond);
            if (((m0 & m) | m1) == m) {
                m = (b == bfirst) ? (m0 & m) : m1;
            } else {
                for (int bit = 0; bit < nbits; ++bit) {
                    const unsigned long long bal = __ballot(valid && ((b >> bit) & 1));
                    m &= ((b >> bit) & 1) ? bal : ~bal;
                }
            }
        }
        const int rank = __popcll(m & ((1ull << lane) - 1ull)), cntb = __popcll(m);
        int pos = 0;
        if (valid) pos = base[b] + rank;
        __builtin_amdgcn_fence(__ATOMIC_RELEASE, "wavefront"); __builtin_amdgcn_wave_barrier();
        if (valid) {
            perm[pos] = (int32_t)i;
            if (rank == 0) base[b] += cntb;
        }
        __builtin_amdgcn_fence(__ATOMIC_RELEASE, "wavefront"); __builtin_amdgcn_wave_barrier();
    }
}

__global__ __launch_bounds__(256) void derive_rows_kernel(double *__restrict__ out, double *__restrict__ cache, const uint8_t *__restrict__ mode,
                                                          uint8_t *__restrict__ dirty, int64_t stride, int K,
                                                          const uint8_t *__restrict__ flags_src, uint8_t *__restrict__ flags_dst) {
    if (flags_dst && blockIdx.x == 0 && blockIdx.y == 0) for (int i = threadIdx.x; i <= K; i += 256) flags_dst[i] = flags_src[i];
    const int k = blockIdx.y;
    const int64_t e = blockIdx.x * 256ll + threadIdx.x;
    const int m = mode[k];
    if (e < stride) {
        double *l = out + (int64_t)(2 * k) * stride, *r = l + stride, *c = cache + (int64_t)k * stride;
        if (m == 0) c[e] = l[e] + r[e];
        else if (m == 1) l[e] = c[e] - r[e];
        else r[e] = c[e] - l[e];
    }
    if (blockIdx.x == 0 && threadIdx.x == 0) { dirty[k] = 0; if (k == 0) dirty[DPMM_MAX_CLUSTERS_K] = 0; }
}
hipError_t launch_derive_rows(double *out, double *cache, const uint8_t *mode, uint8_t *dirty, int64_t stride, int K, const uint8_t *flags_src,
                              uint8_t *flags_dst, hipStream_t s) {
    DPMM_LAUNCH(derive_rows_kernel, dim3((unsigned)((stride + 255) / 256), K), dim3(256), 0, s, out, cache, mode, dirty, stride, K, flags_src, flags_dst);
    return hipGetLastError();
}

#define DPMM_TILE_DISPATCH(tile, CALL512, CALL2048) do { if ((tile) == 512) { CALL512; } else { CALL2048; } } while (0)
static inline int sort_nt(int64_t n, const SortBufs &b) { return (int)((n + b.tile - 1) / b.tile); }
template <int TILE>
static inline void launch_hist(const int32_t *bins, int64_t n, int nbins, int nt, int32_t *tile_cnt, int32_t *fast_total, uint16_t *prev_lab, uint8_t *dirty,
                               hipStream_t s, int32_t *tile_spec = nullptr, int32_t *spec_bins = nullptr, int64_t first = 0, uint64_t seed = 0, uint32_t epoch = 0) {
    if (tile_spec && nbins <= STEP_SPEC_MAX_BINS)
        DPMM_LAUNCH((hist_kernel<TILE, 8, true>), dim3((nt + 7) / 8), dim3(512), 16 * nbins * sizeof(int), s, bins, n, nbins, nt, tile_cnt, fast_total, prev_lab, dirty,
                    tile_spec, spec_bins, first, seed, epoch);
    else if (nbins <= 1024) DPMM_LAUNCH((hist_kernel<TILE, 8, false>), dim3((nt + 7) / 8), dim3(512), 8 * nbins * sizeof(int), s, bins, n, nbins, nt, tile_cnt, fast_total, prev_lab, dirty,
                                        (int32_t *)nullptr, (int32_t *)nullptr, (int64_t)0, (uint64_t)0, 0u);
// ... 600 lines not shown
            }
            if (ok) {
                const int64_t d = d0 + 4 * (int64_t)threadIdx.x;
                if (d < A.D) slab[d] = (double)s0;
                if (d + 1 < A.D) slab[d + 1] = (double)s1;
                if (d + 2 < A.D) slab[d + 2] = (double)s2;
                if (d + 3 < A.D) slab[d + 3] = (double)s3;
            }
        }
    }
}

hipError_t launch_mult_stats_u8(const StatsArgs &a, const uint8_t *X8, int64_t ld8, hipStream_t s) {
    const int grid = a.max_items < 1 ? 1 : a.max_items;
    DPMM_LAUNCH(mult_stats_u8_kernel, dim3(grid), dim3(256), 0, s, a, X8, ld8);
    DPMM_LAUNCH(mult_reduce_kernel, dim3((unsigned)((a.packed_stride + 255) / 256), a.nbins), dim3(256), 0, s, a);
    return hipGetLastError();
}

int64_t mult_slab_stride(int D) { return D; }

hipError_t launch_mult_reduce(const StatsArgs &a, hipStream_t s) {
    DPMM_LAUNCH(mult_reduce_kernel, dim3((unsigned)((a.packed_stride + 255) / 256), a.nbins), dim3(256), 0, s, a);
    return hipGetLastError();
}

hipError_t launch_mult_stats(const StatsArgs &a, hipStream_t s) {
    const int grid = a.max_items < 1 ? 1 : a.max_items;
    DPMM_LAUNCH(mult_stats_kernel, dim3(grid), dim3(256), 0, s, a);
    DPMM_LAUNCH(mult_reduce_kernel, dim3((unsigned)((a.packed_stride + 255) / 256), a.nbins), dim3(256), 0, s, a);
    return hipGetLastError();
}

static void launch_scatter(const int32_t *bins, const StatsArgs &a, int nt, hipStream_t s) {
    const StepStarts none{};
    int32_t *b = const_cast<int32_t *>(bins);
    DPMM_TILE_DISPATCH(a.sb.tile,
        DPMM_LAUNCH((scatter_kernel<512, false>), dim3(nt), dim3(64), a.nbins * sizeof(int), s, b, a.n, a.nbins, nt, a.sb.tile_hist, a.sb.bin_start, a.sb.perm, none),
        DPMM_LAUNCH((scatter_kernel<2048, false>), dim3(nt), dim3(64), a.nbins * sizeof(int), s, b, a.n, a.nbins, nt, a.sb.tile_hist, a.sb.bin_start, a.sb.perm, none));
}
hipError_t launch_step_scan_scatter(int32_t *bins, const StatsArgs &a, int derive, int force_all, int fused_starts, const StepReset *rs, hipStream_t s) {
    const int nt = sort_nt(a.n, a.sb);
    if (rs) DPMM_LAUNCH(scan_tiles_step_kernel, dim3(a.nbins), dim3(256), 0, s, a.sb.tile_cnt, a.sb.tile_spec, a.sb.tile_hist, nt, a.sb.bin_total, a.sb.fast_total,
                        rs->global_counts, rs->flags, rs->K, rs->cside);
    else DPMM_LAUNCH(scan_tiles_kernel, dim3(a.nbins), dim3(256), 0, s, a.sb.tile_cnt, a.sb.tile_hist, nt, a.sb.bin_total);
    if ((fused_starts || rs) && nt > 0) {
        const StepStarts st{a.sb.bin_total, a.sb.bin_sel, a.chunk, a.sb.bin_start, a.sb.item_start, a.sb.perm_total, a.sb.fast_total,
                            derive ? a.sb.cmode : (uint8_t *)nullptr, a.sb.cdirty, force_all,
                            rs ? rs->flags : (const uint8_t *)nullptr, rs ? a.sb.spec_bins : (const int32_t *)nullptr, a.sb.tile_cnt};
        const size_t lds = a.nbins * sizeof(int) + (size_t)(((a.nbins >> 1) + 3) & ~3);
        DPMM_TILE_DISPATCH(a.sb.tile,
            DPMM_LAUNCH((scatter_kernel<512, true>), dim3(nt), dim3(64), lds, s, bins, a.n, a.nbins, nt, a.sb.tile_hist, a.sb.bin_start, a.sb.perm, st),
            DPMM_LAUNCH((scatter_kernel<2048, true>), dim3(nt), dim3(64), lds, s, bins, a.n, a.nbins, nt, a.sb.tile_hist, a.sb.bin_start, a.sb.perm, st));
        return hipGetLastError();
    }
    DPMM_LAUNCH(starts_step_kernel, dim3(1), dim3(256), 0, s, a.sb.bin_total, a.sb.bin_sel, a.nbins, a.chunk, a.sb.bin_start, a.sb.item_start,
                a.sb.perm_total, a.sb.fast_total, derive ? a.sb.cmode : (uint8_t *)nullptr, a.sb.cdirty, force_all);
    launch_scatter(bins, a, nt, s);
    return hipGetLastError();
}
hipError_t launch_sort_finish(const int32_t *bins, const StatsArgs &a, hipStream_t s) {
    const int nt = sort_nt(a.n, a.sb);
    DPMM_LAUNCH(starts_kernel, dim3(1), dim3(256), 0, s, a.sb.bin_total, a.sb.bin_sel, a.nbins, a.chunk,
                       a.sb.bin_start, a.sb.item_start, a.sb.perm_total);
    if (nt > 0) launch_scatter(bins, a, nt, s);
    return hipGetLastError();
}

}
```

### include/dpmm_hip_debug.h

```cpp
#ifndef DPMM_HIP_DEBUG_H
#define DPMM_HIP_DEBUG_H

#include "dpmm_hip.h"

#ifdef __cplusplus
extern "C" {
#endif

int dpmm_debug_loglik(dpmm_ctx *ctx, float *out);
int dpmm_debug_subloglik(dpmm_ctx *ctx, float *out);

int dpmm_debug_niw_draw_inputs(dpmm_ctx *ctx, uint32_t epoch, int K, const int32_t *slot_of_cluster, double *A, double *xi);

int dpmm_debug_ref_bracket(dpmm_ctx *ctx, int64_t cluster, float c_override, float *q_hi, float *q);
int dpmm_debug_pair_ball(dpmm_ctx *ctx, float *pd, float *sn);
int dpmm_debug_pair_ball_sn2(dpmm_ctx *ctx, float *sn2);
int dpmm_debug_norm_cert_points(dpmm_ctx *ctx, int enable, uint8_t *flags);
int dpmm_debug_bracket_big(dpmm_ctx *ctx, float *aref, uint32_t *tile_flags);
int dpmm_debug_mult_draws_ahead(dpmm_ctx *ctx, long long *used);

int dpmm_last_kernel_ms(dpmm_ctx *ctx, float *sweep_ms, float *suffstats_ms);
int dpmm_last_sweep_parts_ms(dpmm_ctx *ctx, float *out3);
int dpmm_last_sweep_work(dpmm_ctx *ctx, uint64_t *out16);
int dpmm_last_comm_ms(dpmm_ctx *ctx, float *counts_ms, float *rows_ms);

int dpmm_debug_counters(dpmm_ctx *ctx, int64_t *out, int n);
int dpmm_debug_sort_tables(dpmm_ctx *ctx, int32_t *perm, int32_t *bin_total, int32_t *bin_start, int32_t *perm_total);
int dpmm_debug_set_prelaunch_hook(void (*fn)(void *), void *arg);

#ifdef __cplusplus
}
#endif
#endif
```

Baseline: 736.4.

## Fuse per-tile bin histogram counting into the NIW sweep kernels

The lean and sub sweep kernels now count the new bin labels per sort tile while they write them. The following statistics step can then skip its separate histogram pass over all N labels when the counts are still valid. The scatter kernel zeroes the count tables for the next sweep, and every label-mutating API call invalidates the fused counts. This saves one full read of the label array per iteration, at the cost of atomic counting inside the sweep, a host sync when the descriptor changes, and more complex invalidation state.

```diff
diff --git a/dpmmsubclusters.jl_amd/binding.py b/dpmmsubclusters.jl_amd/binding.py
--- a/dpmmsubclusters.jl_amd/binding.py
+++ b/dpmmsubclusters.jl_amd/binding.py
@@ -76,6 +76,7 @@
     ("dpmm_last_kernel_ms", ctypes.c_int, [ctypes.c_void_p, _c_f32p, _c_f32p]),
     ("dpmm_debug_counters", ctypes.c_int, [ctypes.c_void_p, ctypes.POINTER(ctypes.c_int64), ctypes.c_int]),
     ("dpmm_debug_sort_tables", ctypes.c_int, [ctypes.c_void_p, ctypes.c_void_p, ctypes.c_void_p, ctypes.c_void_p, ctypes.c_void_p]),
+    ("dpmm_debug_sort_marks", ctypes.c_int, [ctypes.c_void_p, ctypes.c_void_p, ctypes.c_void_p, ctypes.c_void_p, ctypes.c_void_p]),
     ("dpmm_debug_set_prelaunch_hook", ctypes.c_int, [ctypes.c_void_p, ctypes.c_void_p]),
     ("dpmm_init_labels_from", ctypes.c_int, [ctypes.c_void_p, ctypes.c_int, ctypes.c_int, ctypes.c_uint32]),
     ("dpmm_set_option", ctypes.c_int, [ctypes.c_void_p, ctypes.c_int, ctypes.c_double]),
@@ -1357,6 +1358,14 @@
         self._chk(self._lib.dpmm_debug_sort_tables(self._h, perm.ctypes.data, tot.ctypes.data, start.ctypes.data, ptot.ctypes.data))
         return perm[:int(ptot[0])].copy(), tot, start
 
+    def debug_sort_marks(self):
+        cnt = np.zeros(4, np.int64)
+        self._chk(self._lib.dpmm_debug_sort_marks(self._h, None, None, None, cnt.ctypes.data))
+        nt = int(cnt[2])
+        th = np.empty((2 * self.K, max(nt, 1)), np.int32); pl = np.empty(max(self.n, 1), np.uint16); dirty = np.empty(self.K, np.uint8)
+        self._chk(self._lib.dpmm_debug_sort_marks(self._h, th.ctypes.data, pl.ctypes.data, dirty.ctypes.data, cnt.ctypes.data))
+        return th[:, :nt], pl[:self.n], dirty, [int(v) for v in cnt]
+
     def debug_counters(self):
         out = (ctypes.c_int64 * 4)()
         self._chk(self._lib.dpmm_debug_counters(self._h, out, 4))
diff --git a/dpmmsubclusters.jl_amd/csrc/dpmm_api.cpp b/dpmmsubclusters.jl_amd/csrc/dpmm_api.cpp
--- a/dpmmsubclusters.jl_amd/csrc/dpmm_api.cpp
+++ b/dpmmsubclusters.jl_amd/csrc/dpmm_api.cpp
@@ -71,6 +71,8 @@
     float min2 = 0.f;
     bool accumulated = false;
 };
+
+constexpr int DPMM_CHAIN_DEFAULT = 0x7fffffff & ~(8 | 32 | 64);
 
 struct dpmm_ctx {
     int prior = 0, D = 0, device = 0;
@@ -320,7 +322,15 @@
     int sp_cooldown = 0;
     int opt_b3 = 1;
     bool have_b3 = false;
-    int opt_chain = 0x7fffffff & ~(8 | 32);
+    bool cnt_counted = false;
+    int cnt_nbins = 0, cnt_nt = 0;
+    int64_t cnt_n = 0;
+    bool cnt_totals_stale = false;
+    int64_t cnt_dirty = 0;
+    DevBuf<SweepCount> d_cnt_desc;
+    SweepCount h_cnt_desc{};
+    int64_t dbg_hist_passes = 0, dbg_swept_passes = 0;
+    int opt_chain = DPMM_CHAIN_DEFAULT;
     DevBuf<uint8_t> d_cert_rec;
     int opt_lean_norm_cert = 1;
     int opt_pair_ball = 1;
@@ -427,6 +437,13 @@
     return code;
 }
 
+static inline void cnt_invalidate(dpmm_ctx *c) {
+    if (!c->cnt_counted) return;
+    c->cnt_counted = false;
+    c->cnt_totals_stale = true;
+    c->cnt_dirty = std::max(c->cnt_dirty, (int64_t)c->cnt_nbins * (int64_t)c->cnt_nt);
+}
+
 template <class Buf>
 static int regrow(dpmm_ctx *c, Buf &buf, size_t need, const char *who, const char *what, size_t floor = 0) {
     const size_t cap = grow_capacity(need, floor);
@@ -676,6 +693,7 @@
     const size_t nbmax = 2 * DPMM_MAX_CLUSTERS;
     CHK_CREATE(c->sort_mem.tile_hist.alloc(sizeof(int32_t) * nbmax * (size_t)std::max(1, c->nt_sort)));
     CHK_CREATE(c->sort_mem.tile_cnt.alloc(sizeof(int32_t) * nbmax * (size_t)std::max(1, c->nt_sort)));
+    CHK_CREATE(hipMemsetAsync(c->sort_mem.tile_cnt, 0, sizeof(int32_t) * nbmax * (size_t)std::max(1, c->nt_sort), c->stream));
     CHK_CREATE(c->sort_mem.tile_spec.alloc(sizeof(int32_t) * (size_t)STEP_SPEC_MAX_BINS * (size_t)std::max(1, c->nt_sort)));
     CHK_CREATE(c->sort_mem.spec_bins.alloc(sizeof(int32_t) * nalloc));
     CHK_CREATE(c->sort_mem.fast_total.alloc(sizeof(int32_t) * nbmax * FAST_TOTAL_STRIDE));
@@ -943,6 +961,7 @@
     if (!c) return DPMM_EINVAL;
     if (init_clusters < 1 || init_clusters > DPMM_MAX_CLUSTERS) return fail(c, DPMM_ELIMIT, "init_clusters out of range");
     HIPCHK(c, hipSetDevice(c->device));
+    cnt_invalidate(c);
     if (c->n > 0) HIPCHK(c, launch_init_labels(c->dbins, c->n, c->first, init_clusters, 0, c->seed, epoch, c->stream));
     c->have_labels = true;
     c->rows_full_K = -1;
@@ -953,6 +972,7 @@
     if (!c) return DPMM_EINVAL;
     if (first_label < 1 || init_clusters < 1 || first_label - 1 + init_clusters > DPMM_MAX_CLUSTERS) return fail(c, DPMM_ELIMIT, "init_clusters / first_label out of range");
     HIPCHK(c, hipSetDevice(c->device));
+    cnt_invalidate(c);
     if (c->n > 0) HIPCHK(c, launch_init_labels(c->dbins, c->n, c->first, init_clusters, first_label - 1, c->seed, epoch, c->stream));
     c->have_labels = true;
     c->rows_full_K = -1;
@@ -970,6 +990,7 @@
     hipError_t e = hipSuccess;
     if (labels) e = hipMemcpyAsync(tmp, labels, sizeof(int64_t) * c->n, hipMemcpyHostToDevice, c->stream);
     if (e == hipSuccess && sub) e = hipMemcpyAsync(tmp + c->n, sub, sizeof(int64_t) * c->n, hipMemcpyHostToDevice, c->stream);
+    cnt_invalidate(c);
     if (e == hipSuccess) e = launch_bins_from_i64(c->dbins, labels ? tmp.get() : nullptr, sub ? tmp + c->n : nullptr, c->n, c->stream);
     if (e == hipSuccess) e = sync_stream(c, c->stream);
     if (e != hipSuccess) { c->err = std::string("dpmm_set_labels: ") + hipGetErrorString(e); rc = DPMM_EHIP; }
@@ -1342,6 +1363,31 @@
     const bool parts = (c->opt_timing & 8) != 0 && (c->opt_timing & 1) != 0;
     if (parts && !c->ev_part[0]) for (auto &e : c->ev_part) HIPCHK(c, hipEventCreate(&e));
     NiwLabelStore ls{true};
+    SweepCount cnt{};
+    const SweepCount *cntp = nullptr;
+    const bool was_counted = c->cnt_counted;
+    cnt_invalidate(c);
+    {
+        const int nbins = 2 * c->K;
+        const bool fold_reset = (c->opt_chain & 8) != 0 && (c->n >= 4000000 || (c->opt_chain & 32) != 0) && nbins <= STEP_SPEC_MAX_BINS;
+#ifdef DPMM_STAMPS
+        const bool stamps = true;
+#else
+        const bool stamps = false;
+#endif
+        if ((c->opt_chain & 64) != 0 && !stamps && !was_counted && c->cnt_dirty == 0 && !c->cnt_totals_stale && !comm_attached(c) && !fold_reset && c->n > 0 &&
+            c->sb.tile_cnt && c->sb.fast_total && (c->sb.tile == SORT_TILE || c->sb.tile == SORT_TILE_SMALL)) {
+            cnt.tile_cnt = c->sb.tile_cnt; cnt.fast_total = c->sb.fast_total; cnt.prev_lab = c->sb.prev_lab; cnt.dirty = c->sb.prev_lab ? c->sb.cdirty : nullptr;
+            cnt.nt = (int)((c->n + c->sb.tile - 1) / c->sb.tile); cnt.tile_shift = c->sb.tile == SORT_TILE ? 11 : 9; cnt.nbins = nbins;
+            cntp = &cnt;
+            if (use_lean && memcmp(&cnt, &c->h_cnt_desc, sizeof(cnt)) != 0) {
+                if (!c->d_cnt_desc) HIPCHK(c, c->d_cnt_desc.alloc(sizeof(SweepCount)));
+                HIPCHK(c, sync_stream(c, c->stream));
+                HIPCHK(c, hipMemcpy(c->d_cnt_desc, &cnt, sizeof(cnt), hipMemcpyHostToDevice));
+                c->h_cnt_desc = cnt;
+            }
+        }
+    }
     if (use_lean) {
         const size_t hw = hard_list_words(c->n);
         uint32_t *mine = c->d_hard + (size_t)c->hard_flip * hw, *other = c->d_hard + (size_t)(c->hard_flip ^ 1) * hw;
@@ -1359,15 +1405,20 @@
 #ifndef DPMM_STAMPS
         al_args.cert_points = c->d_cert_rec;
 #endif
-        HIPCHK(c, launch_niw_lean(al_args, mine, need2, other, al ? c->sb.bin_start : nullptr, al ? c->perm_nbins : 0, need3, c->sweep_grid, c->stream));
+        HIPCHK(c, launch_niw_lean(al_args, mine, need2, other, al ? c->sb.bin_start : nullptr, al ? c->perm_nbins : 0, need3, c->sweep_grid, c->stream, cntp));
         if (parts) HIPCHK(c, hipEventRecord(c->ev_part[0], c->stream));
         ls.tile_list = mine;
         ls.list_len = c->h_hard;
     }
-    HIPCHK(c, launch_niw_sweep(c->NB, a, c->sweep_grid, c->stream, ls));
+    NiwSweepArgs la = a;
+#ifndef DPMM_STAMPS
+    if (cntp && ls.tile_list) la.count_tables = c->d_cnt_desc;
+#endif
+    HIPCHK(c, launch_niw_sweep(c->NB, la, c->sweep_grid, c->stream, ls));
     if (parts) HIPCHK(c, hipEventRecord(c->ev_part[1], c->stream));
     c->have_parts = parts ? (use_lean ? 2 : 1) : 0;
-    if (!ls.tile_list) HIPCHK(c, launch_niw_sub(a, nullptr, nullptr, c->sweep_grid, c->stream));
+    if (!ls.tile_list) HIPCHK(c, launch_niw_sub(a, nullptr, nullptr, c->sweep_grid, c->stream, cntp));
+    if (cntp) { c->cnt_counted = true; c->cnt_nbins = cnt.nbins; c->cnt_nt = cnt.nt; c->cnt_n = c->n; }
     return DPMM_OK;
 }
 
@@ -1554,6 +1605,7 @@
     if (!c->undo_pending) return DPMM_OK;
     c->undo_pending = false;
     const uint8_t *flags = reinterpret_cast<const uint8_t *>(c->d_out.get()) + sizeof(double) * 2 * (size_t)c->K * (size_t)c->packed_stride;
+    cnt_invalidate(c);
     HIPCHK(c, launch_niw_undo_reset(c->dbins, c->n, c->K, flags, c->d_cside, c->stream));
     return DPMM_OK;
 }
@@ -1594,7 +1646,22 @@
     if (with_reset && c->n > 0) {
         const bool fold_reset = (c->opt_chain & 8) != 0 && (c->n >= 4000000 || (c->opt_chain & 32) != 0) && nbins <= STEP_SPEC_MAX_BINS &&
                                 c->sb.tile_spec != nullptr && c->sb.spec_bins != nullptr;
-        HIPCHK(c, launch_step_hist(c->dbins, c->n, nbins, c->sb, c->stream, fold_reset ? 1 : 0, c->first, c->seed, reset_epoch));
+        const int nt_now = (int)((c->n + c->sb.tile - 1) / c->sb.tile);
+        const bool swept = c->cnt_counted && c->cnt_nbins == nbins && c->cnt_nt == nt_now && c->cnt_n == c->n && !fold_reset;
+        if (swept) { c->cnt_counted = false; c->dbg_swept_passes += 1; }
+        else {
+            cnt_invalidate(c);
+            if (c->cnt_totals_stale) HIPCHK(c, hipMemsetAsync(c->sb.fast_total, 0, sizeof(int32_t) * 2 * DPMM_MAX_CLUSTERS * FAST_TOTAL_STRIDE, c->stream));
+            c->cnt_totals_stale = false;
+            c->dbg_hist_passes += 1;
+            HIPCHK(c, launch_step_hist(c->dbins, c->n, nbins, c->sb, c->stream, fold_reset ? 1 : 0, c->first, c->seed, reset_epoch));
+        }
+        const bool clear_cnt = (c->opt_chain & 64) != 0 && !comm_attached(c);
+        {
+            const int64_t extent = (int64_t)nbins * nt_now;
+            if (!clear_cnt) c->cnt_dirty = std::max(c->cnt_dirty, extent);
+            else if (extent >= c->cnt_dirty) c->cnt_dirty = 0;
+        }
         const long long *gc = nullptr;
         if (comm_attached(c) && !one_coll) {
             HIPCHK(c, launch_widen_counts(c->sb.fast_total, FAST_TOTAL_STRIDE, c->d_counts64, nbins, c->stream));
@@ -1606,10 +1673,12 @@
         derive = c->opt_derive != 0;
         const int force_all = (c->cache_force || c->cache_K != c->K) ? 1 : 0;
         const StepReset rs{gc, flags, c->K, one_coll ? c->d_cside : nullptr, c->first, c->seed, reset_epoch};
-        HIPCHK(c, launch_step_scan_scatter(c->dbins, a, derive ? 1 : 0, force_all, c->opt_chain & 1, fold_reset ? &rs : nullptr, c->stream));
+        HIPCHK(c, launch_step_scan_scatter(c->dbins, a, derive ? 1 : 0, force_all, c->opt_chain & 1, fold_reset ? &rs : nullptr, c->stream, clear_cnt ? 1 : 0));
         if (derive) { c->sel_all_ones = 0; c->cache_force = false; c->cache_K = c->K; }
     } else {
         if (c->n > 0) {
+            cnt_invalidate(c);
+            c->cnt_dirty = std::max(c->cnt_dirty, (int64_t)nbins * (int64_t)((c->n + c->sb.tile - 1) / c->sb.tile));
             HIPCHK(c, launch_sort_by_bin(c->dbins, c->n, nbins, c->sb, c->stream));
         } else {
             HIPCHK(c, hipMemsetAsync(c->sb.bin_total, 0, sizeof(int32_t) * nbins, c->stream));
@@ -1690,6 +1759,8 @@
     const int nbins = 2 * c->K;
     if (c->n == 0) { for (int b = 0; b < nbins; ++b) counts[b] = 0; return DPMM_OK; }
     if (int rc = ensure_pinned(c, sizeof(int32_t) * nbins)) return rc;
+    cnt_invalidate(c);
+    c->cnt_dirty = std::max(c->cnt_dirty, (int64_t)nbins * (int64_t)((c->n + c->sb.tile - 1) / c->sb.tile));
     HIPCHK(c, launch_sort_by_bin(c->dbins, c->n, nbins, c->sb, c->stream));
     HIPCHK(c, launch_copy_bytes(c->h_pin, c->sb.bin_total, sizeof(int32_t) * nbins, c->stream));
     HIPCHK(c, sync_stream(c, c->stream));
@@ -1961,6 +2032,19 @@
     HIPCHK(c, hipMemcpy(bin_total, c->sb.bin_total, sizeof(int32_t) * 2 * (size_t)c->K, hipMemcpyDeviceToHost));
     HIPCHK(c, hipMemcpy(bin_start, c->sb.bin_start, sizeof(int32_t) * (2 * (size_t)c->K + 1), hipMemcpyDeviceToHost));
     HIPCHK(c, hipMemcpy(perm_total, c->sb.perm_total, sizeof(int32_t), hipMemcpyDeviceToHost));
+    return DPMM_OK;
+}
+
+int dpmm_debug_sort_marks(dpmm_ctx *c, int32_t *tile_hist, uint16_t *prev_lab, uint8_t *dirty, int64_t *counters) {
+    if (!c) return DPMM_EINVAL;
+    if (!c->have_perm || c->K < 1) return fail(c, DPMM_ESTATE, "no statistics pass has sorted the points yet");
+    HIPCHK(c, hipSetDevice(c->device));
+    HIPCHK(c, hipStreamSynchronize(c->stream));
+    const int64_t nt = (c->n + c->sb.tile - 1) / c->sb.tile;
+    if (tile_hist) HIPCHK(c, hipMemcpy(tile_hist, c->sb.tile_hist, sizeof(int32_t) * 2 * (size_t)c->K * (size_t)nt, hipMemcpyDeviceToHost));
+    if (prev_lab && c->sb.prev_lab) HIPCHK(c, hipMemcpy(prev_lab, c->sb.prev_lab, sizeof(uint16_t) * (size_t)c->n, hipMemcpyDeviceToHost));
+    if (dirty) HIPCHK(c, hipMemcpy(dirty, c->sb.cdirty, (size_t)c->K, hipMemcpyDeviceToHost));
+    if (counters) { counters[0] = c->dbg_hist_passes; counters[1] = c->dbg_swept_passes; counters[2] = nt; counters[3] = c->h_hard ? (int64_t)c->h_hard[0] : 0; }
     return DPMM_OK;
 }
 
@@ -2528,6 +2612,7 @@
     if (!idx || !new_idx) return fail(c, DPMM_EINVAL, "null index list");
     HIPCHK(c, hipSetDevice(c->device));
     if (int rc = upload_idx(c, idx, new_idx, n, DPMM_MAX_CLUSTERS)) return rc;
+    cnt_invalidate(c);
     if (c->n > 0) HIPCHK(c, launch_split(c->dbins, c->n, c->first, c->d_small, n, c->seed, epoch, c->stream));
     c->rows_full_K = -1;
     return DPMM_OK;
@@ -2540,6 +2625,7 @@
     if (!idx || !new_idx) return fail(c, DPMM_EINVAL, "null index list");
     HIPCHK(c, hipSetDevice(c->device));
     if (int rc = upload_idx(c, idx, new_idx, n, DPMM_MAX_CLUSTERS)) return rc;
+    cnt_invalidate(c);
     if (c->n > 0) HIPCHK(c, launch_merge(c->dbins, c->n, c->d_small, n, c->stream));
     c->rows_full_K = -1;
     return DPMM_OK;
@@ -2564,6 +2650,7 @@
     HIPCHK(c, sync_stream(c, c->stream));
     memcpy(c->h_pin, map.data(), sizeof(int32_t) * map.size());
     HIPCHK(c, launch_copy_bytes(c->d_small, c->h_pin, sizeof(int32_t) * map.size(), c->stream));
+    cnt_invalidate(c);
     if (c->n > 0) HIPCHK(c, launch_remap(c->dbins, c->n, c->d_small, c->stream));
     c->rows_full_K = -1;
     return DPMM_OK;
@@ -2577,6 +2664,7 @@
         if (n == 0) return DPMM_OK;
         if (int rc = upload_idx(c, idx, nullptr, n, DPMM_MAX_CLUSTERS)) return rc;
     }
+    cnt_invalidate(c);
     if (c->n > 0) HIPCHK(c, launch_reset_sub(c->dbins, c->n, c->first, idx ? c->d_small : nullptr, idx ? n : 0, c->seed, epoch, c->stream));
     c->rows_full_K = -1;
     return DPMM_OK;
@@ -2636,6 +2724,7 @@
     if (int rc = smart_check(c, cluster)) return rc;
     if (!c->d_proj) return fail(c, DPMM_ESTATE, "dpmm_smart_project has not been called");
     HIPCHK(c, hipSetDevice(c->device));
+    cnt_invalidate(c);
     if (c->n > 0) HIPCHK(c, launch_smart_assign(c->dbins, c->d_proj, c->n, (int)(cluster - 1), m_lo, m_hi, c->stream));
     return DPMM_OK;
 }
@@ -2721,7 +2810,7 @@
         case DPMM_OPT_PAIR_BALL: c->opt_pair_ball = value != 0; if (!c->opt_pair_ball) c->have_pb = false; return DPMM_OK;
         case DPMM_OPT_LEAN_NORM_CERT: c->opt_lean_norm_cert = (value == 2 || value == 3) ? value : (value != 0); c->cert_cool = 0; c->cert_fb = false; return DPMM_OK;
         case DPMM_OPT_LEAN_DIRECTION: c->opt_lean_dir = value != 0; c->lean_off = 0; c->lean_backoff = 15; c->lean_ran = false; return DPMM_OK;
-        case DPMM_OPT_CHAIN_FUSION: c->opt_chain = value < 0 ? (0x7fffffff & ~(8 | 32)) : (int)value; return DPMM_OK;
+        case DPMM_OPT_CHAIN_FUSION: c->opt_chain = value < 0 ? DPMM_CHAIN_DEFAULT : (int)value; return DPMM_OK;
         case DPMM_OPT_LEAN_TILES: c->opt_lean = value != 0; c->lean_off = 0; c->lean_backoff = 15; c->lean_ran = false; return DPMM_OK;
         case DPMM_OPT_B3_SUBLABELS: c->opt_b3 = value != 0; if (!c->opt_b3) c->have_b3 = false; return DPMM_OK;
         case DPMM_OPT_DIRECTION_SCREEN:
@@ -2743,6 +2832,8 @@
                     tsp.alloc(sizeof(int32_t) * (size_t)STEP_SPEC_MAX_BINS * (size_t)std::max(1, nt)) != hipSuccess)
                     return fail(c, DPMM_EHIP, "DPMM_OPT_SORT_TILE: out of device memory for the 512-point tile tables");
                 c->sort_mem.tile_hist = std::move(th); c->sort_mem.tile_cnt = std::move(tc); c->sort_mem.tile_spec = std::move(tsp);
+                HIPCHK(c, hipMemsetAsync(c->sort_mem.tile_cnt, 0, sizeof(int32_t) * nbmax * (size_t)std::max(1, nt), c->stream));
+                cnt_invalidate(c); c->cnt_dirty = 0;
                 sort_view(c);
                 c->nt_sort = nt; c->sort_tile_min = t;
             }
@@ -3382,6 +3473,7 @@
     if (d_labels) if (int rc = check_device_extent(c, fn, "d_labels", d_labels, bytes, sizeof(int64_t))) return rc;
     if (d_sub) if (int rc = check_device_extent(c, fn, "d_sub", d_sub, bytes, sizeof(int64_t))) return rc;
     if (d_labels || d_sub) {
+        cnt_invalidate(c);
         HIPCHK(c, launch_bins_from_i64(c->dbins, d_labels, d_sub, c->n, c->stream));
         HIPCHK(c, sync_stream(c, c->stream));
     }
diff --git a/dpmmsubclusters.jl_amd/csrc/dpmm_kernels.h b/dpmmsubclusters.jl_amd/csrc/dpmm_kernels.h
--- a/dpmmsubclusters.jl_amd/csrc/dpmm_kernels.h
+++ b/dpmmsubclusters.jl_amd/csrc/dpmm_kernels.h
@@ -25,6 +25,17 @@
 enum NiwScreens : int {
     NIW_SCR_ON = 1,
     NIW_SCR_DIR_FIRST = 2,
+};
+
+struct SweepCount {
+    int32_t *tile_cnt;
+    int32_t *fast_total;
+    uint16_t *prev_lab;
+    uint8_t *dirty;
+    int nt;
+    int tile_shift;
+    int nbins;
+    int pad;
 };
 
 struct NiwSweepArgs {
@@ -77,6 +88,7 @@
     union {
         unsigned long long *dbg;
         uint8_t *cert_points;
+        const SweepCount *count_tables;
     };
     int queue_rounds;
     int prio;
@@ -124,9 +136,10 @@
     return 16 * (cap + 2) + 16 * cap + (size_t)REFB_WORDS * cap + 3 * cap * (size_t)B3_WORDS + 3 * cap * (size_t)B3_DVEC + niw_pair_ball_floats(cap < (size_t)PB_MAXK ? cap : (size_t)PB_MAXK);
 }
 hipError_t launch_niw_b3_debug(const NiwSweepArgs &a, float *out, hipStream_t s);
-hipError_t launch_niw_sub(const NiwSweepArgs &a, const uint32_t *list, uint32_t *count_out, int grid, hipStream_t s);
+hipError_t launch_niw_sub(const NiwSweepArgs &a, const uint32_t *list, uint32_t *count_out, int grid, hipStream_t s, const SweepCount *cnt = nullptr);
+constexpr int SWEEP_COUNT_LDS_BINS = 512;
 constexpr int NIW_LEAN_MAX_BINS = 256;
-hipError_t launch_niw_lean(const NiwSweepArgs &a, uint32_t *list, uint32_t *need2, uint32_t *other_list, const int32_t *bin_start, int nbins, uint32_t *need3, int grid, hipStream_t s);
+hipError_t launch_niw_lean(const NiwSweepArgs &a, uint32_t *list, uint32_t *need2, uint32_t *other_list, const int32_t *bin_start, int nbins, uint32_t *need3, int grid, hipStream_t s, const SweepCount *cnt = nullptr);
 hipError_t launch_niw_direction(const float *Rp, const float *mup, const float *cst, int D, int K, uint32_t *frag, float *cons, hipStream_t s);
 
 struct MultSweepArgs {
@@ -684,7 +697,7 @@
 hipError_t launch_niw_undo_reset(int32_t *bins, int64_t n, int K, const uint8_t *flags, const uint8_t *cside, hipStream_t s);
 struct StatsArgs;
 hipError_t launch_sort_finish(const int32_t *bins, const StatsArgs &a, hipStream_t s);
-hipError_t launch_step_scan_scatter(int32_t *bins, const StatsArgs &a, int derive, int force_all, int fused_starts, const StepReset *rs, hipStream_t s);
+hipError_t launch_step_scan_scatter(int32_t *bins, const StatsArgs &a, int derive, int force_all, int fused_starts, const StepReset *rs, hipStream_t s, int clear_cnt = 0);
 hipError_t launch_derive_rows(double *out, double *cache, const uint8_t *mode, uint8_t *dirty, int64_t stride, int K, const uint8_t *flags_src,
                               uint8_t *flags_dst, hipStream_t s);
 
diff --git a/dpmmsubclusters.jl_amd/csrc/niw_device.h b/dpmmsubclusters.jl_amd/csrc/niw_device.h
--- a/dpmmsubclusters.jl_amd/csrc/niw_device.h
+++ b/dpmmsubclusters.jl_amd/csrc/niw_device.h
@@ -180,4 +180,39 @@
     return K >= 64 ? far : far & ((1ull << K) - 1ull);
 }
 
-}
+__device__ __forceinline__ void sweep_count_tile(const SweepCount &C, int p, int bin, bool valid, int lane, int *tot, unsigned q) {
+    const bool inr = valid && (unsigned)bin < (unsigned)C.nbins;
+    if (C.prev_lab && valid) {
+        const unsigned z = inr ? (unsigned)bin >> 1 : 0xFFFFu;
+        if (z != q) {
+            if (inr) C.dirty[z] = 1;
+            if (q < DPMM_MAX_CLUSTERS_K) C.dirty[q] = 1;
+            C.prev_lab[p] = (uint16_t)z;
+        }
+    }
+    const int64_t at = (int64_t)bin * C.nt + (p >> C.tile_shift);
+    const unsigned key = (unsigned)at;
+    auto add = [&](int c) {
+        atomicAdd(C.tile_cnt + at, c);
+        if (tot) atomicAdd(&tot[bin], c);
+        else atomicAdd(&C.fast_total[bin * FAST_TOTAL_STRIDE], c);
+    };
+    unsigned long long rem = __ballot(inr);
+#pragma unroll 1
+    for (int r = 0; r < 4 && rem; ++r) {
+        const int leader = __ffsll((long long)rem) - 1;
+        const unsigned k0 = (unsigned)__builtin_amdgcn_readlane((int)key, leader);
+        const unsigned long long m = __ballot(inr && key == k0);
+        if (lane == leader) add(__popcll(m));
+        rem &= ~m;
+    }
+    if ((rem >> lane) & 1ull) add(1);
+}
+__device__ __forceinline__ void sweep_count_flush(const SweepCount &C, const int *tot, int tid, int nthreads) {
+    for (int b = tid; b < C.nbins; b += nthreads) {
+        const int v = tot[b];
+        if (v) atomicAdd(&C.fast_total[b * FAST_TOTAL_STRIDE], v);
+    }
+}
+
+}
diff --git a/dpmmsubclusters.jl_amd/csrc/niw_lean.hip b/dpmmsubclusters.jl_amd/csrc/niw_lean.hip
--- a/dpmmsubclusters.jl_amd/csrc/niw_lean.hip
+++ b/dpmmsubclusters.jl_amd/csrc/niw_lean.hip
@@ -80,8 +80,14 @@
 }
 
 
-template <bool LISTED>
-__global__ __launch_bounds__(256, 2) void niw_sub_kernel(NiwSweepArgs A, const uint32_t *__restrict__ list, uint32_t *__restrict__ count_out) {
+template <bool LISTED, bool COUNT>
+__device__ __forceinline__ void niw_sub_body(NiwSweepArgs A, const uint32_t *__restrict__ list, uint32_t *__restrict__ count_out, const SweepCount &C) {
+    __shared__ int cnt_tot[COUNT ? SWEEP_COUNT_LDS_BINS : 1];
+    int *const ctot = COUNT && C.nbins <= SWEEP_COUNT_LDS_BINS ? cnt_tot : nullptr;
+    if constexpr (COUNT) {
+        for (int e = threadIdx.x; e < SWEEP_COUNT_LDS_BINS; e += 256) cnt_tot[e] = 0;
+        __syncthreads();
+    }
     if (LISTED && count_out && blockIdx.x == 0 && threadIdx.x == 0) *count_out = list[0];
     const int lane = threadIdx.x & 63, ci = lane & 15, g = lane >> 4;
     const bool use_order = A.order != nullptr && *A.order_total == (int32_t)A.n;
@@ -102,14 +108,18 @@
     span_words((int64_t)wave_id + nwaves, sa2, sb2);
     int64_t t_next = pack_span(sa, sb);
     int nx_p = -1, nx_z = -1;
+    int nx_raw = -1;
     if (t_next >= 0) {
         const int64_t pos = (t_next >> 7) + lane;
-        if (lane < (int)(t_next & 127)) { nx_p = use_order ? A.order[pos] : (int)pos; nx_z = label_of(A.bins[nx_p]); }
+        if (lane < (int)(t_next & 127)) { nx_p = use_order ? A.order[pos] : (int)pos; nx_raw = A.bins[nx_p]; nx_z = label_of(nx_raw); }
     }
     for (int64_t idx = wave_id; idx < count; idx += nwaves) {
         t_next = pack_span(sa2, sb2);
         const int myp32 = nx_p;
         const int z = nx_z;
+        [[maybe_unused]] const int raw = nx_raw;
+        unsigned pl = 0u;
+        if constexpr (COUNT) { if (C.prev_lab && myp32 >= 0) pl = C.prev_lab[myp32]; }
         int pf_p = -1, pf_bin = -1;
         const bool has_next = t_next >= 0 && lane < (int)(t_next & 127);
         bool bin_asked = false;
@@ -144,15 +154,35 @@
             if (z == k) { b0 = bl; b1 = br; }
             nw_b3 += 2;
         }
-        if (z >= 0) A.bins[myp32] = 2 * z + draw2(b0, b1, u_sub);
+        const int nbin = z >= 0 ? 2 * z + draw2(b0, b1, u_sub) : raw;
+        if (z >= 0) A.bins[myp32] = nbin;
+        if constexpr (COUNT) sweep_count_tile(C, myp32, nbin, myp32 >= 0, lane, ctot, pl);
         if (!bin_asked && has_next) pf_bin = A.bins[pf_p];
         nx_p = pf_p; nx_z = has_next ? label_of(pf_bin) : -1;
+        if constexpr (COUNT) nx_raw = has_next ? pf_bin : -1;
         asm volatile("" : "+v"(nx_z));
     }
+    if constexpr (COUNT) {
+        __syncthreads();
+        if (ctot) sweep_count_flush(C, ctot, threadIdx.x, 256);
+    }
     if (A.work && lane == 0) A.work[DPMM_WORK_SLOTS + (size_t)wave_id * DPMM_WORK_PER_WAVE + 7] += (unsigned long long)nw_b3 << 32;
 }
-hipError_t launch_niw_sub(const NiwSweepArgs &a, const uint32_t *list, uint32_t *count_out, int grid, hipStream_t s) {
+template <bool LISTED>
+__global__ __launch_bounds__(256, 2) void niw_sub_kernel(NiwSweepArgs A, const uint32_t *__restrict__ list, uint32_t *__restrict__ count_out) {
+    niw_sub_body<LISTED, false>(A, list, count_out, SweepCount{});
+}
+template <bool LISTED>
+__global__ __launch_bounds__(256, 2) void niw_sub_cnt_kernel(NiwSweepArgs A, const uint32_t *__restrict__ list, uint32_t *__restrict__ count_out, SweepCount C) {
+    niw_sub_body<LISTED, true>(A, list, count_out, C);
+}
+hipError_t launch_niw_sub(const NiwSweepArgs &a, const uint32_t *list, uint32_t *count_out, int grid, hipStream_t s, const SweepCount *cnt) {
     if (!a.tail || a.n <= 0) return hipErrorInvalidValue;
+    if (cnt) {
+        if (list) DPMM_LAUNCH(niw_sub_cnt_kernel<true>, dim3(grid), dim3(256), 0, s, a, list, count_out, *cnt);
+        else DPMM_LAUNCH(niw_sub_cnt_kernel<false>, dim3(grid), dim3(256), 0, s, a, list, count_out, *cnt);
+        return hipGetLastError();
+    }
     if (list) DPMM_LAUNCH(niw_sub_kernel<true>, dim3(grid), dim3(256), 0, s, a, list, count_out);
     else DPMM_LAUNCH(niw_sub_kernel<false>, dim3(grid), dim3(256), 0, s, a, list, count_out);
     return hipGetLastError();
@@ -201,9 +231,9 @@
 #else
 #define LSTAMP(var)
 #endif
-template <bool DIR>
+template <bool DIR, bool COUNT>
 __device__ __forceinline__ void niw_lean_body(NiwSweepArgs A, uint32_t *__restrict__ list, uint32_t *__restrict__ need2, uint32_t *__restrict__ other_list,
-                                              const int32_t *__restrict__ bin_start, int nbins, uint32_t *__restrict__ need3) {
+                                              const int32_t *__restrict__ bin_start, int nbins, uint32_t *__restrict__ need3, const SweepCount &C) {
     if (other_list && blockIdx.x == 0 && threadIdx.x == 0) other_list[0] = 0u;
 #ifdef DPMM_STAMPS
     unsigned long long T_x = 0, T_conv = 0, T_br = 0, T_scr = 0, T_u = 0, T_p2 = 0, T_tot = 0; int ntl = 0;
@@ -234,6 +264,9 @@
     }
     constexpr int MAXB = NIW_LEAN_MAX_BINS;
     __shared__ int tstart_s[MAXB + 2], bstart_s[MAXB + 2], wsum_s[4];
+    __shared__ int cnt_tot[COUNT ? SWEEP_COUNT_LDS_BINS : 1];
+    int *const ctot = COUNT && C.nbins <= SWEEP_COUNT_LDS_BINS ? cnt_tot : nullptr;
+    if constexpr (COUNT) for (int e = threadIdx.x; e < SWEEP_COUNT_LDS_BINS; e += 256) cnt_tot[e] = 0;
     const bool aligned = bin_start != nullptr && use_order && nbins >= 1 && nbins <= MAXB && bin_start[nbins] == (int32_t)A.n;
     const int nb = aligned ? nbins : 1;
     {
@@ -471,9 +504,17 @@
             if (lane == 0) { const uint32_t at = atomicAdd(&list[0], 1u); list[1 + 2 * at] = (uint32_t)c_p0; list[2 + 2 * at] = (uint32_t)c_cn; }
             if (!bin_asked && lane < n_cn) pf_bin = A.bins[pf_p];
         } else {
+            unsigned pl = 0u;
+            if constexpr (COUNT) { if (C.prev_lab && valid) pl = C.prev_lab[myp32]; }
             float bl, br;
             b3_eval(A.tail, K, k0, Z, H, lane, g, bl, br);
+            if constexpr (COUNT) {
+                const int nbin = 2 * k0 + draw2(bl, br, u_sub);
+                if (valid) A.bins[myp32] = nbin;
+                sweep_count_tile(C, myp32, nbin, valid, lane, ctot, pl);
+            } else {
             if (valid) A.bins[myp32] = 2 * k0 + draw2(bl, br, u_sub);
+            }
 #ifndef DPMM_STAMPS
             if (cheap && A.cert_points && valid) A.cert_points[myp32] = 1;
 #endif
@@ -493,6 +534,10 @@
         d[0] = T_x; d[1] = T_conv; d[2] = T_br; d[3] = T_scr; d[4] = T_u; d[5] = T_p2; d[6] = 0; d[7] = T_tot; d[8] = ntl;
     }
 #endif
+    if constexpr (COUNT) {
+        __syncthreads();
+        if (ctot) sweep_count_flush(C, ctot, threadIdx.x, 256);
+    }
     if (A.work && lane == 0) {
         unsigned long long *slot = A.work + DPMM_WORK_SLOTS + (size_t)wave_id * DPMM_WORK_PER_WAVE;
         slot[0] += nw_easy; slot[3] += nw_tail; slot[4] += nw_br; slot[5] += nw_bb; slot[7] += ((unsigned long long)(2 * nw_easy) << 32) + nw_sp;
@@ -510,15 +555,29 @@
 }
 __global__ __launch_bounds__(256, 2) void niw_lean_kernel(NiwSweepArgs A, uint32_t *__restrict__ list, uint32_t *__restrict__ need2, uint32_t *__restrict__ other_list,
                                                          const int32_t *__restrict__ bin_start, int nbins, uint32_t *__restrict__ need3) {
-    niw_lean_body<false>(A, list, need2, other_list, bin_start, nbins, need3);
+    niw_lean_body<false, false>(A, list, need2, other_list, bin_start, nbins, need3, SweepCount{});
 }
 __global__ __launch_bounds__(256, 2) void niw_lean_kernel_dir(NiwSweepArgs A, uint32_t *__restrict__ list, uint32_t *__restrict__ need2, uint32_t *__restrict__ other_list,
                                                              const int32_t *__restrict__ bin_start, int nbins, uint32_t *__restrict__ need3) {
-    niw_lean_body<true>(A, list, need2, other_list, bin_start, nbins, need3);
-}
-hipError_t launch_niw_lean(const NiwSweepArgs &a, uint32_t *list, uint32_t *need2, uint32_t *other_list, const int32_t *bin_start, int nbins, uint32_t *need3, int grid, hipStream_t s) {
+    niw_lean_body<true, false>(A, list, need2, other_list, bin_start, nbins, need3, SweepCount{});
+}
+__global__ __launch_bounds__(256, 2) void niw_lean_kernel_cnt(NiwSweepArgs A, uint32_t *__restrict__ list, uint32_t *__restrict__ need2, uint32_t *__restrict__ other_list,
+                                                             const int32_t *__restrict__ bin_start, int nbins, uint32_t *__restrict__ need3, SweepCount C) {
+    niw_lean_body<false, true>(A, list, need2, other_list, bin_start, nbins, need3, C);
+}
+__global__ __launch_bounds__(256, 2) void niw_lean_kernel_dir_cnt(NiwSweepArgs A, uint32_t *__restrict__ list, uint32_t *__restrict__ need2, uint32_t *__restrict__ other_list,
+                                                                 const int32_t *__restrict__ bin_start, int nbins, uint32_t *__restrict__ need3, SweepCount C) {
+    niw_lean_body<true, true>(A, list, need2, other_list, bin_start, nbins, need3, C);
+}
+hipError_t launch_niw_lean(const NiwSweepArgs &a, uint32_t *list, uint32_t *need2, uint32_t *other_list, const int32_t *bin_start, int nbins, uint32_t *need3, int grid, hipStream_t s,
+                           const SweepCount *cnt) {
     if (!a.tail || a.n <= 0 || !list) return hipErrorInvalidValue;
     if (nbins > NIW_LEAN_MAX_BINS) { bin_start = nullptr; nbins = 0; }
+    if (cnt) {
+        if (niw_dir_screen(a) && a.K >= 3) DPMM_LAUNCH(niw_lean_kernel_dir_cnt, dim3(grid), dim3(256), 0, s, a, list, need2, other_list, bin_start, nbins, need3, *cnt);
+        else DPMM_LAUNCH(niw_lean_kernel_cnt, dim3(grid), dim3(256), 0, s, a, list, need2, other_list, bin_start, nbins, need3, *cnt);
+        return hipGetLastError();
+    }
     if (niw_dir_screen(a) && a.K >= 3) DPMM_LAUNCH(niw_lean_kernel_dir, dim3(grid), dim3(256), 0, s, a, list, need2, other_list, bin_start, nbins, need3);
     else DPMM_LAUNCH(niw_lean_kernel, dim3(grid), dim3(256), 0, s, a, list, need2, other_list, bin_start, nbins, need3);
     return hipGetLastError();
diff --git a/dpmmsubclusters.jl_amd/csrc/niw_sweep.hip b/dpmmsubclusters.jl_amd/csrc/niw_sweep.hip
--- a/dpmmsubclusters.jl_amd/csrc/niw_sweep.hip
+++ b/dpmmsubclusters.jl_amd/csrc/niw_sweep.hip
@@ -1532,7 +1532,15 @@
                     if (z == kk) { b0 = bl; b1 = br; }
                     nw_b3l += 2;
                 }
-                if (valid) A.bins[myp] = 2 * z + draw2(b0, b1, u_sub);
+                const int nbin = 2 * z + draw2(b0, b1, u_sub);
+                if (valid) A.bins[myp] = nbin;
+#ifndef DPMM_STAMPS
+                if (A.count_tables) {
+                    const SweepCount C = *A.count_tables;
+                    const unsigned pl = (C.prev_lab && valid) ? C.prev_lab[myp] : 0u;
+                    sweep_count_tile(C, (int)myp, nbin, valid, lane, nullptr, pl);
+                }
+#endif
             }
             nx_p = pf_p; nx_bin = pf_bin; nx_tile = tnext < tile_sent ? tnext : -1;
             l_pos = nl_pos; l_end = nl_end;
diff --git a/dpmmsubclusters.jl_amd/csrc/suffstats.hip b/dpmmsubclusters.jl_amd/csrc/suffstats.hip
--- a/dpmmsubclusters.jl_amd/csrc/suffstats.hip
+++ b/dpmmsubclusters.jl_amd/csrc/suffstats.hip
@@ -382,6 +382,7 @@
     uint8_t *mode; const uint8_t *dirty; int force_all;
     const uint8_t *reset_flags; const int32_t *spec_bins;
     const int32_t *tile_cnt;
+    int32_t *clear_cnt;
 };
 template <int TILE, bool STEP>
 __global__ __launch_bounds__(64) void scatter_kernel(int32_t *bins, int64_t n, int nbins, int nt,
@@ -494,6 +495,8 @@
         }
         __builtin_amdgcn_fence(__ATOMIC_RELEASE, "wavefront"); __builtin_amdgcn_wave_barrier();
     }
+    if (st.clear_cnt)
+        for (int b = lane; b < nbins; b += 64) st.clear_cnt[(int64_t)b * nt + blockIdx.x] = 0;
 }
 
 __global__ __launch_bounds__(256) void derive_rows_kernel(double *__restrict__ out, double *__restrict__ cache, const uint8_t *__restrict__ mode,
@@ -1160,14 +1163,15 @@
     return hipGetLastError();
 }
 
-static void launch_scatter(const int32_t *bins, const StatsArgs &a, int nt, hipStream_t s) {
-    const StepStarts none{};
+static void launch_scatter(const int32_t *bins, const StatsArgs &a, int nt, hipStream_t s, int clear_cnt = 0) {
+    StepStarts none{};
+    if (clear_cnt) none.clear_cnt = a.sb.tile_cnt;
     int32_t *b = const_cast<int32_t *>(bins);
     DPMM_TILE_DISPATCH(a.sb.tile,
         DPMM_LAUNCH((scatter_kernel<512, false>), dim3(nt), dim3(64), a.nbins * sizeof(int), s, b, a.n, a.nbins, nt, a.sb.tile_hist, a.sb.bin_start, a.sb.perm, none),
         DPMM_LAUNCH((scatter_kernel<2048, false>), dim3(nt), dim3(64), a.nbins * sizeof(int), s, b, a.n, a.nbins, nt, a.sb.tile_hist, a.sb.bin_start, a.sb.perm, none));
 }
-hipError_t launch_step_scan_scatter(int32_t *bins, const StatsArgs &a, int derive, int force_all, int fused_starts, const StepReset *rs, hipStream_t s) {
+hipError_t launch_step_scan_scatter(int32_t *bins, const StatsArgs &a, int derive, int force_all, int fused_starts, const StepReset *rs, hipStream_t s, int clear_cnt) {
     const int nt = sort_nt(a.n, a.sb);
     if (rs) DPMM_LAUNCH(scan_tiles_step_kernel, dim3(a.nbins), dim3(256), 0, s, a.sb.tile_cnt, a.sb.tile_spec, a.sb.tile_hist, nt, a.sb.bin_total, a.sb.fast_total,
                         rs->global_counts, rs->flags, rs->K, rs->cside);
@@ -1175,7 +1179,8 @@
     if ((fused_starts || rs) && nt > 0) {
         const StepStarts st{a.sb.bin_total, a.sb.bin_sel, a.chunk, a.sb.bin_start, a.sb.item_start, a.sb.perm_total, a.sb.fast_total,
                             derive ? a.sb.cmode : (uint8_t *)nullptr, a.sb.cdirty, force_all,
-                            rs ? rs->flags : (const uint8_t *)nullptr, rs ? a.sb.spec_bins : (const int32_t *)nullptr, a.sb.tile_cnt};
+                            rs ? rs->flags : (const uint8_t *)nullptr, rs ? a.sb.spec_bins : (const int32_t *)nullptr, a.sb.tile_cnt,
+                            clear_cnt ? a.sb.tile_cnt : (int32_t *)nullptr};
         const size_t lds = a.nbins * sizeof(int) + (size_t)(((a.nbins >> 1) + 3) & ~3);
         DPMM_TILE_DISPATCH(a.sb.tile,
             DPMM_LAUNCH((scatter_kernel<512, true>), dim3(nt), dim3(64), lds, s, bins, a.n, a.nbins, nt, a.sb.tile_hist, a.sb.bin_start, a.sb.perm, st),
@@ -1184,7 +1189,7 @@
     }
     DPMM_LAUNCH(starts_step_kernel, dim3(1), dim3(256), 0, s, a.sb.bin_total, a.sb.bin_sel, a.nbins, a.chunk, a.sb.bin_start, a.sb.item_start,
                 a.sb.perm_total, a.sb.fast_total, derive ? a.sb.cmode : (uint8_t *)nullptr, a.sb.cdirty, force_all);
-    launch_scatter(bins, a, nt, s);
+    launch_scatter(bins, a, nt, s, clear_cnt);
     return hipGetLastError();
 }
 hipError_t launch_sort_finish(const int32_t *bins, const StatsArgs &a, hipStream_t s) {
diff --git a/include/dpmm_hip_debug.h b/include/dpmm_hip_debug.h
--- a/include/dpmm_hip_debug.h
+++ b/include/dpmm_hip_debug.h
@@ -26,6 +26,7 @@
 
 int dpmm_debug_counters(dpmm_ctx *ctx, int64_t *out, int n);
 int dpmm_debug_sort_tables(dpmm_ctx *ctx, int32_t *perm, int32_t *bin_total, int32_t *bin_start, int32_t *perm_total);
+int dpmm_debug_sort_marks(dpmm_ctx *ctx, int32_t *tile_hist, uint16_t *prev_lab, uint8_t *dirty, int64_t *counters);
 int dpmm_debug_set_prelaunch_hook(void (*fn)(void *), void *arg);
 
 #ifdef __cplusplus
```

After: 736.3, median of 2. Within noise of the previous version (-0.0%).
